# zhouhang95/ray_tracing_in_one_weekend

Measured on AMD Instinct MI355X. Metric: Mray/s (primary+secondary) at 1920x1080/256spp, higher is better.
Workload: dtype f32

## Files before the change

### include/rtow_mi355x_debug.h

```cpp
#ifndef RTOW_MI355X_DEBUG_H
#define RTOW_MI355X_DEBUG_H

#include "rtow_mi355x.h"

#ifdef __cplusplus
extern "C" {
#endif

#define RT_FLAG_TIME_DEPTHS 4u
#define RT_FLAG_PRODUCTION_KERNELS 8u

int rt_get_depth_timings(RtCtx* ctx, uint32_t max_n, float* isect_ms, float* shade_ms, uint64_t* rays);

int rt_debug_render_parts(const RtCtx* ctx, char* buf, uint32_t cap);

enum RtDebugOption {
    RT_OPT_TREE_PLACEMENT = 0,
    RT_OPT_PRIMARY_LISTS = 1,
    RT_OPT_PIXEL_ORDER = 2,
    RT_OPT_TEXEL_POOL = 3,
    RT_OPT_GRID = 4,
    RT_OPT_GRID_CELL = 5,
    RT_OPT_CHAINS = 6,
    RT_OPT_GENERAL_KERNELS = 7,
    RT_OPT_GENERAL_LDS = 8,
    RT_OPT_QUEUE_SHARDS = 9,
    RT_OPT_ISECT_WORKGROUPS = 10,
    RT_OPT_MATERIALISE_PRIMARIES = 11,
    RT_OPT_MEDIUM_SEARCH = 12,
    RT_OPT_POOL_CHUNK_DELAY_US = 13,
    RT_OPT__COUNT = 14
};
int rt_debug_set_option(RtCtx* ctx, uint32_t option, uint32_t value);
int rt_debug_get_option(const RtCtx* ctx, uint32_t option, uint32_t* value);

typedef struct RtSceneInfo {
    uint32_t n_entries;
    uint32_t n_tree_nodes, tree_depth;
    uint32_t tree_in_lds;
    uint32_t general_kernels;
    uint32_t closest_hit_lds_bytes;
    uint32_t grid;
    uint32_t grid_cells[3];
    uint32_t grid_refs;
    uint32_t grid_always;
    uint32_t grid_lds_bytes;
    float grid_cell_size[3];
    uint32_t general_tables_in_lds;
    uint32_t nest;
} RtSceneInfo;
int rt_debug_scene_info(const RtCtx* ctx, RtSceneInfo* info);

int rt_debug_planar_info(const RtCtx* ctx, uint32_t* n_planar, uint32_t* plane_data_in_lds);
int rt_debug_planar_bounds(const RtQuads* quads, float world_mag, float* box, float* slack);

int rt_debug_grid_build(const RtFlatScene* scene, uint32_t cell_per_mille, uint32_t lds_budget, float grid[8], uint32_t dims[3],
                        uint32_t* cells, uint32_t* n_cells, uint16_t* refs, uint32_t* n_refs, uint32_t large[4], uint32_t* n_large);

int rt_debug_world_bounds(const RtFlatScene* scene, float* prim_box, float* prim_box_padded, float* world_sphere, uint32_t* n_entries,
                          uint32_t* entry_id, float* entry_box_padded, float* entry_bs);

int rt_debug_motion_bounds(const RtCtx* ctx, float* entry_box_padded, float* entry_sphere, uint32_t* entry_id, uint32_t entry_cap, uint32_t* n_entries,
                           float grid[6], uint32_t dims[3], uint32_t* cell_begin, uint32_t* cell_id, uint32_t cell_cap, uint32_t* n_cell_ids);

#ifdef RT_PROFILE_LANES
int rt_debug_lane_stats(unsigned long long* out24, int reset);
#endif

typedef struct RtBounceIO {
    uint32_t n;
    uint32_t depth;
    const float* in_o;
    const float* in_d;
    const uint32_t* in_key;
    int32_t* out_hit;
    float* out_t;
    float* out_radiance;
    float* out_attenuation;
    float* out_o;
    float* out_d;
    uint8_t* out_alive;
    uint32_t flags;
} RtBounceIO;
int rt_debug_bounce(RtCtx* ctx, const RtBounceIO* io);

#define RT_ARITH_SHARED_DIVISION 0u
#define RT_ARITH_SQRT 1u
#define RT_ARITH_TO_I32 2u
#define RT_ARITH_TO_U32 3u
int rt_debug_arithmetic(RtCtx* ctx, uint32_t op, uint32_t n, const float* x, const float* a, float* out);


#ifdef __cplusplus
}
#endif
#endif
```

### ray_tracing_in_one_weekend_amd/_ffi.py

```python
import ctypes as C
import os

_PKG_DIR = os.path.dirname(os.path.abspath(__file__))
GPU_LIB_PATH = os.environ.get("RTOW_GPU_LIB") or os.path.join(_PKG_DIR, "librtow_mi355x.so")
HOST_LIB_PATH = os.path.join(_PKG_DIR, "librtow_host.so")

RT_NO_TEX = 0xFFFFFFFF
ERR_INVALID, ERR_DEVICE, ERR_NOMEM, ERR_UNSUPPORTED, ERR_STATE = 1, 2, 3, 4, 5
FLAG_BRUTE_FORCE = 1
FLAG_RUSSIAN_ROULETTE = 2
FLAG_TIME_DEPTHS = 4
FLAG_PRODUCTION_KERNELS = 8
RTH_INVALID = 0xFFFFFFFF

(MAT_EMISSION, MAT_DIFFUSE, MAT_LAMBERT, MAT_METAL, MAT_DIELECTRIC, MAT_ISOTROPIC, MAT_OREN_NAYAR,
 MAT_BURLEY_DIFFUSE, MAT_ROUGH_PLASTIC, MAT_DISNEY_DIFFUSE, MAT_DISNEY_METAL, MAT_DISNEY_SHEEN,
 MAT_DISNEY_CLEARCOAT) = range(13)
TEX_CONSTANT, TEX_CHECKER, TEX_PERLIN, TEX_IMAGE = range(4)
RECT_YZ, RECT_XZ, RECT_XY = range(3)
XF_TRANSLATE, XF_ROTATE_Y = range(2)
NO_XFORM = 0xFFFFFFFF
SKY_GRADIENT, SKY_BLACK, SKY_ENV = range(3)

_f = C.POINTER(C.c_float)
_u8 = C.POINTER(C.c_uint8)
_u16 = C.POINTER(C.c_uint16)
_u32 = C.POINTER(C.c_uint32)
_u64 = C.POINTER(C.c_uint64)


class RtFlatScene(C.Structure):
    _fields_ = [
        ("n_spheres", C.c_uint32),
        ("sph_cx", _f), ("sph_cy", _f), ("sph_cz", _f), ("sph_r", _f), ("sph_mat", _u32),
        ("n_rects", C.c_uint32),
        ("rect_axis", _u8), ("rect_min", _f), ("rect_max", _f), ("rect_mat", _u32),
        ("n_xforms", C.c_uint32),
        ("xf_type", _u8), ("xf_param", _f), ("xf_parent", _u32), ("sph_xform", _u32), ("rect_xform", _u32),
        ("n_media", C.c_uint32),
        ("med_neg_inv_density", _f), ("med_mat", _u32), ("sph_medium", _u32), ("rect_medium", _u32), ("med_xform", _u32),
        ("n_materials", C.c_uint32),
        ("mat_type", _u8), ("mat_color", _f), ("mat_p0", _f), ("mat_p1", _f), ("mat_p2", _f), ("mat_p3", _f),
        ("mat_tex0", _u32), ("mat_tex1", _u32),
        ("n_textures", C.c_uint32),
        ("tex_type", _u8), ("tex_color0", _f), ("tex_color1", _f), ("tex_scale", _f), ("tex_aux", _u32),
        ("n_perlin", C.c_uint32),
        ("perlin_vec", _f), ("perlin_perm", _u16),
        ("n_images", C.c_uint32),
        ("img_w", _u32), ("img_h", _u32), ("img_offset", _u64), ("texels", _f), ("n_texel_floats", C.c_uint64),
        ("sky_type", C.c_uint32), ("sky_image", C.c_uint32),
    ]


class RtCamera(C.Structure):
    _fields_ = [("origin", C.c_float * 3), ("horizontal", C.c_float * 3), ("vertical", C.c_float * 3),
                ("lower_left_corner", C.c_float * 3)]


class RtLens(C.Structure):
    _fields_ = [("lens_radius", C.c_float), ("focus_dist", C.c_float)]


class RtMotion(C.Structure):
    _fields_ = [("n_moving", C.c_uint32), ("sphere", C.POINTER(C.c_uint32)), ("center1", C.POINTER(C.c_float)),
                ("shutter_open", C.c_float), ("shutter_close", C.c_float)]


class RtQuads(C.Structure):
    _fields_ = [("n", C.c_uint32), ("q", C.POINTER(C.c_float)), ("u", C.POINTER(C.c_float)), ("v", C.POINTER(C.c_float)),
                ("kind", C.POINTER(C.c_uint8)), ("mat", C.POINTER(C.c_uint32))]


PLANAR_QUAD, PLANAR_TRIANGLE = 0, 1
PLANAR_MIN_SIN2 = 2.0 ** -20
PLANAR_REACH = 16.0


class RtParams(C.Structure):
    _fields_ = [("nx", C.c_uint32), ("ny", C.c_uint32), ("spp", C.c_uint32), ("max_depth", C.c_int32),
                ("seed", C.c_uint64), ("shard_band", C.c_uint32), ("shard_count", C.c_uint32),
                ("shard_id", C.c_uint32), ("spp_slice", C.c_uint32), ("flags", C.c_uint32), ("reserved", C.c_uint32)]


class RtStats(C.Structure):
    _fields_ = [("n_paths", C.c_uint64), ("n_rays", C.c_uint64), ("n_rays_secondary", C.c_uint64),
                ("n_texture_fetches", C.c_uint64), ("n_bad_dir", C.c_uint64), ("seconds_total", C.c_double),
                ("seconds_trace", C.c_double), ("seconds_device", C.c_double), ("bytes_algorithmic", C.c_uint64),
                ("bytes_trace_algorithmic", C.c_uint64), ("n_trace_launches", C.c_uint32), ("n_slices", C.c_uint32),
                ("rays_per_depth", C.c_uint64 * 64)]

    def as_dict(self):
        d = {k: getattr(self, k) for k, _ in self._fields_ if k != "rays_per_depth"}
        d["rays_per_depth"] = list(self.rays_per_depth)
        return d


class RtBounceIO(C.Structure):
    _fields_ = [("n", C.c_uint32), ("depth", C.c_uint32), ("in_o", _f), ("in_d", _f), ("in_key", _u32),
                ("out_hit", C.POINTER(C.c_int32)), ("out_t", _f), ("out_radiance", _f), ("out_attenuation", _f),
                ("out_o", _f), ("out_d", _f), ("out_alive", _u8), ("flags", C.c_uint32)]


RtProgressFn = C.CFUNCTYPE(None, C.c_void_p, C.c_uint32, C.c_uint32, C.POINTER(C.c_uint8), C.c_uint32, C.c_uint32)

MULTI_COPY_GATHER = 1
(OPT_TREE_PLACEMENT, OPT_PRIMARY_LISTS, OPT_PIXEL_ORDER, OPT_TEXEL_POOL, OPT_GRID, OPT_GRID_CELL, OPT_CHAINS,
 OPT_GENERAL_KERNELS, OPT_GENERAL_LDS, OPT_QUEUE_SHARDS, OPT_ISECT_WORKGROUPS, OPT_MATERIALISE_PRIMARIES, OPT_MEDIUM_SEARCH, OPT_POOL_CHUNK_DELAY_US) = range(14)
OPT_NAMES = {"tree_placement": OPT_TREE_PLACEMENT, "primary_lists": OPT_PRIMARY_LISTS, "pixel_order": OPT_PIXEL_ORDER,
             "texel_pool": OPT_TEXEL_POOL, "grid": OPT_GRID, "grid_cell": OPT_GRID_CELL, "chains": OPT_CHAINS,
             "general_kernels": OPT_GENERAL_KERNELS, "general_lds": OPT_GENERAL_LDS, "queue_shards": OPT_QUEUE_SHARDS,
             "isect_workgroups": OPT_ISECT_WORKGROUPS, "materialise_primaries": OPT_MATERIALISE_PRIMARIES,
             "medium_search": OPT_MEDIUM_SEARCH, "pool_chunk_delay_us": OPT_POOL_CHUNK_DELAY_US}


class RtSceneInfo(C.Structure):
    _fields_ = [("n_entries", C.c_uint32), ("n_tree_nodes", C.c_uint32), ("tree_depth", C.c_uint32), ("tree_in_lds", C.c_uint32),
                ("general_kernels", C.c_uint32), ("closest_hit_lds_bytes", C.c_uint32), ("grid", C.c_uint32),
                ("grid_cells", C.c_uint32 * 3), ("grid_refs", C.c_uint32), ("grid_always", C.c_uint32),
                ("grid_lds_bytes", C.c_uint32), ("grid_cell_size", C.c_float * 3), ("general_tables_in_lds", C.c_uint32), ("nest", C.c_uint32)]

    def as_dict(self):
        d = {k: getattr(self, k) for k, _ in self._fields_ if k not in ("grid_cells", "grid_cell_size")}
        d["grid_cells"], d["grid_cell_size"] = list(self.grid_cells), [float(x) for x in self.grid_cell_size]
        return d


EXPECTED_ABI = 11
GPU_SYMBOLS = ["rt_abi_version", "rt_build_id", "rt_ctx_create", "rt_ctx_destroy", "rt_last_error", "rt_scene_upload",
               "rt_shard_rows", "rt_shard_row_to_image_row", "rt_prepare", "rt_render", "rt_render_device", "rt_debug_bounce", "rt_debug_arithmetic",
               "rt_get_depth_timings", "rt_set_progress", "rt_host_alloc", "rt_host_free", "rt_debug_set_option", "rt_debug_get_option",
               "rt_debug_scene_info", "rt_debug_grid_build", "rt_debug_world_bounds", "rt_debug_render_parts", "rt_multi_create", "rt_multi_create_ex", "rt_multi_destroy", "rt_multi_device_count",
               "rt_multi_last_error", "rt_multi_scene_upload", "rt_multi_render", "rt_deinterleave_bands", "rt_set_lens", "rt_multi_set_lens",
               "rt_set_motion", "rt_multi_set_motion", "rt_debug_motion_bounds",
               "rt_set_quads", "rt_multi_set_quads", "rt_debug_planar_info", "rt_debug_planar_bounds"]
HOST_SYMBOLS = ["rth_last_error", "rth_register_image", "rth_rng_reseed", "rth_scene_build", "rth_scene_new",
                "rth_tex_constant", "rth_tex_checker", "rth_tex_perlin", "rth_tex_image", "rth_material",
                "rth_sphere", "rth_rect", "rth_gbox", "rth_translate", "rth_rotate_y", "rth_constant_medium", "rth_hitable_bbox", "rth_set_sky", "rth_set_camera", "rth_scene_finish", "rth_scene_flat",
                "rth_scene_camera", "rth_scene_sphere_name", "rth_scene_free", "rth_png_write", "rth_output_file_name",
                "rth_set_camera_lens", "rth_scene_lens",
                "rth_moving_sphere", "rth_set_camera_shutter", "rth_scene_motion",
                "rth_quad", "rth_triangle", "rth_scene_quads"]

_gpu_lib = None
_host_lib = None


class GpuLibraryMissing(RuntimeError):
    pass


def load_gpu_library():
    global _gpu_lib
    if _gpu_lib is not None:
        return _gpu_lib
    if not os.path.exists(GPU_LIB_PATH):
        raise GpuLibraryMissing(
            f"{GPU_LIB_PATH} is missing: build it with `python -c 'import __graft_entry__ as g; g.build()'` "
            "(hipcc --offload-arch=gfx950).  There is no CPU fallback for the render path.")
    lib = C.CDLL(GPU_LIB_PATH)
    vp = C.c_void_p
    lib.rt_abi_version.restype = C.c_uint32
    if lib.rt_abi_version() != EXPECTED_ABI:
        raise GpuLibraryMissing(f"{GPU_LIB_PATH} has ABI version {lib.rt_abi_version()}, this package expects {EXPECTED_ABI}: "
                                "rebuild it (python -c 'import __graft_entry__ as g; g.build()')")
    lib.rt_build_id.restype = C.c_char_p
    lib.rt_ctx_create.argtypes = [C.c_int, C.POINTER(vp)]
    lib.rt_ctx_create.restype = C.c_int
    lib.rt_ctx_destroy.argtypes = [vp]
    lib.rt_ctx_destroy.restype = None
    lib.rt_last_error.argtypes = [vp]
    lib.rt_last_error.restype = C.c_char_p
    lib.rt_scene_upload.argtypes = [vp, C.POINTER(RtFlatScene)]
    lib.rt_scene_upload.restype = C.c_int
    lib.rt_shard_rows.argtypes = [C.c_uint32] * 4
    lib.rt_shard_rows.restype = C.c_uint32
    lib.rt_shard_row_to_image_row.argtypes = [C.c_uint32] * 4
    lib.rt_shard_row_to_image_row.restype = C.c_uint32
    lib.rt_prepare.argtypes = [vp, C.POINTER(RtParams)]
    lib.rt_prepare.restype = C.c_int
    lib.rt_render.argtypes = [vp, C.POINTER(RtCamera), C.POINTER(RtParams), _f, _u8, C.POINTER(RtStats)]
    lib.rt_render.restype = C.c_int
    lib.rt_render_device.argtypes = [vp, C.POINTER(RtCamera), C.POINTER(RtParams), vp, vp, C.POINTER(RtStats)]
    lib.rt_render_device.restype = C.c_int
    lib.rt_get_depth_timings.argtypes = [vp, C.c_uint32, _f, _f, _u64]
    lib.rt_get_depth_timings.restype = C.c_int
    lib.rt_debug_bounce.argtypes = [vp, C.POINTER(RtBounceIO)]
    lib.rt_debug_bounce.restype = C.c_int
    lib.rt_debug_arithmetic.argtypes = [vp, C.c_uint32, C.c_uint32, C.POINTER(C.c_float), C.POINTER(C.c_float), C.POINTER(C.c_float)]
    lib.rt_debug_arithmetic.restype = C.c_int
    lib.rt_set_progress.argtypes = [vp, RtProgressFn, vp]
    lib.rt_set_progress.restype = C.c_int
    lib.rt_set_lens.argtypes = [vp, C.POINTER(RtLens)]
    lib.rt_set_lens.restype = C.c_int
    lib.rt_multi_set_lens.argtypes = [vp, C.POINTER(RtLens)]
    lib.rt_multi_set_lens.restype = C.c_int
    lib.rt_set_motion.argtypes = [vp, C.POINTER(RtMotion)]
    lib.rt_set_motion.restype = C.c_int
    lib.rt_multi_set_motion.argtypes = [vp, C.POINTER(RtMotion)]
    lib.rt_multi_set_motion.restype = C.c_int
    lib.rt_debug_motion_bounds.argtypes = [vp, vp, vp, vp, C.c_uint32, C.POINTER(C.c_uint32), C.c_float * 6, C.c_uint32 * 3, vp, vp, C.c_uint32,
                                           C.POINTER(C.c_uint32)]
    lib.rt_debug_motion_bounds.restype = C.c_int
    lib.rt_set_quads.argtypes = [vp, C.POINTER(RtQuads)]
    lib.rt_set_quads.restype = C.c_int
    lib.rt_multi_set_quads.argtypes = [vp, C.POINTER(RtQuads)]
    lib.rt_multi_set_quads.restype = C.c_int
    lib.rt_debug_planar_info.argtypes = [vp, C.POINTER(C.c_uint32), C.POINTER(C.c_uint32)]
    lib.rt_debug_planar_info.restype = C.c_int
    lib.rt_debug_planar_bounds.argtypes = [C.POINTER(RtQuads), C.c_float, vp, vp]
    lib.rt_debug_planar_bounds.restype = C.c_int
    lib.rt_host_alloc.argtypes = [C.c_size_t]
    lib.rt_host_alloc.restype = vp
    lib.rt_host_free.argtypes = [vp]
    lib.rt_host_free.restype = None
    lib.rt_debug_set_option.argtypes = [vp, C.c_uint32, C.c_uint32]
    lib.rt_debug_set_option.restype = C.c_int
    lib.rt_debug_get_option.argtypes = [vp, C.c_uint32, _u32]
    lib.rt_debug_get_option.restype = C.c_int
    lib.rt_debug_scene_info.argtypes = [vp, C.POINTER(RtSceneInfo)]
    lib.rt_debug_scene_info.restype = C.c_int
    lib.rt_debug_render_parts.argtypes = [vp, C.c_char_p, C.c_uint32]
    lib.rt_debug_render_parts.restype = C.c_int
    lib.rt_debug_grid_build.argtypes = [C.POINTER(RtFlatScene), C.c_uint32, C.c_uint32, C.c_float * 8, C.c_uint32 * 3, _u32, _u32, _u16, _u32,
                                        C.c_uint32 * 4, _u32]
    lib.rt_debug_grid_build.restype = C.c_int
    lib.rt_debug_world_bounds.argtypes = [C.POINTER(RtFlatScene), _f, _f, _f, _u32, _u32, _f, _f]
    lib.rt_debug_world_bounds.restype = C.c_int
    lib.rt_multi_create.argtypes = [C.POINTER(C.c_int), C.c_int, C.POINTER(vp)]
    lib.rt_multi_create.restype = C.c_int
    lib.rt_multi_create_ex.argtypes = [C.POINTER(C.c_int), C.c_int, C.c_uint32, C.POINTER(vp)]
    lib.rt_multi_create_ex.restype = C.c_int
    lib.rt_multi_destroy.argtypes = [vp]
    lib.rt_multi_destroy.restype = None
    lib.rt_multi_device_count.argtypes = [vp]
    lib.rt_multi_device_count.restype = C.c_int
    lib.rt_multi_last_error.argtypes = [vp]
    lib.rt_multi_last_error.restype = C.c_char_p
    lib.rt_multi_scene_upload.argtypes = [vp, C.POINTER(RtFlatScene)]
    lib.rt_multi_scene_upload.restype = C.c_int
    lib.rt_multi_render.argtypes = [vp, C.POINTER(RtCamera), C.POINTER(RtParams), _f, _u8, C.POINTER(RtStats)]
    lib.rt_multi_render.restype = C.c_int
    lib.rt_deinterleave_bands.argtypes = [vp, vp, C.c_uint32, C.c_uint32, C.c_uint32, C.c_uint32, vp, vp, vp]
    lib.rt_deinterleave_bands.restype = C.c_int
    _gpu_lib = lib
    return lib


def load_host_library():
    global _host_lib
    if _host_lib is not None:
        return _host_lib
    if not os.path.exists(HOST_LIB_PATH):
        raise RuntimeError(f"{HOST_LIB_PATH} is missing: run __graft_entry__.build()")
    lib = C.CDLL(HOST_LIB_PATH)
    vp = C.c_void_p
    f3 = C.c_float * 3
    lib.rth_last_error.restype = C.c_char_p
    lib.rth_register_image.argtypes = [C.c_char_p, C.c_uint32, C.c_uint32, _f]
    lib.rth_register_image.restype = C.c_int
    lib.rth_rng_reseed.argtypes = [C.c_uint64]
    lib.rth_rng_reseed.restype = None
    lib.rth_scene_build.argtypes = [C.c_char_p, C.c_float, C.POINTER(vp)]
    lib.rth_scene_build.restype = C.c_int
    lib.rth_scene_new.argtypes = [C.POINTER(vp)]
    lib.rth_scene_new.restype = C.c_int
    lib.rth_tex_constant.argtypes = [vp, f3]
    lib.rth_tex_constant.restype = C.c_uint32
    lib.rth_tex_checker.argtypes = [vp, f3, f3]
    lib.rth_tex_checker.restype = C.c_uint32
    lib.rth_tex_perlin.argtypes = [vp, C.c_float]
    lib.rth_tex_perlin.restype = C.c_uint32
    lib.rth_tex_image.argtypes = [vp, C.c_char_p]
    lib.rth_tex_image.restype = C.c_uint32
    lib.rth_material.argtypes = [vp, C.c_uint32, C.c_uint32, C.c_uint32, f3, C.c_float * 4]
    lib.rth_material.restype = C.c_uint32
    lib.rth_sphere.argtypes = [vp, f3, C.c_float, C.c_uint32, C.c_char_p]
    lib.rth_sphere.restype = C.c_uint32
    lib.rth_rect.argtypes = [vp, C.c_uint32, f3, f3, C.c_uint32]
    lib.rth_rect.restype = C.c_uint32
    lib.rth_gbox.argtypes = [vp, f3, f3, C.c_uint32]
    lib.rth_gbox.restype = C.c_uint32
    lib.rth_translate.argtypes = [vp, C.c_uint32, f3]
    lib.rth_translate.restype = C.c_uint32
    lib.rth_rotate_y.argtypes = [vp, C.c_uint32, C.c_float]
    lib.rth_rotate_y.restype = C.c_uint32
    lib.rth_constant_medium.argtypes = [vp, C.c_uint32, C.c_float, C.c_uint32]
    lib.rth_constant_medium.restype = C.c_uint32
    lib.rth_hitable_bbox.argtypes = [vp, C.c_uint32, C.c_float * 6]
    lib.rth_hitable_bbox.restype = C.c_int
    lib.rth_set_sky.argtypes = [vp, C.c_uint32, C.c_char_p]
    lib.rth_set_sky.restype = C.c_int
    lib.rth_set_camera.argtypes = [vp, f3, f3, f3, C.c_float, C.c_float]
    lib.rth_set_camera.restype = C.c_int
    lib.rth_scene_finish.argtypes = [vp, C.c_int]
    lib.rth_scene_finish.restype = C.c_int
    lib.rth_scene_flat.argtypes = [vp]
    lib.rth_scene_flat.restype = C.POINTER(RtFlatScene)
    lib.rth_scene_camera.argtypes = [vp, C.POINTER(RtCamera)]
    lib.rth_scene_camera.restype = C.c_int
    lib.rth_set_camera_lens.argtypes = [vp, f3, f3, f3, C.c_float, C.c_float, C.c_float, C.c_float]
    lib.rth_set_camera_lens.restype = C.c_int
    lib.rth_scene_lens.argtypes = [vp, C.POINTER(RtLens)]
    lib.rth_scene_lens.restype = C.c_int
# ... 23 lines not shown
```

### ray_tracing_in_one_weekend_amd/api.py

```python
import ctypes as C

import numpy as np

from . import _ffi
from ._ffi import RtBounceIO, RtCamera, RtFlatScene, RtLens, RtMotion, RtParams, RtQuads, RtStats


class RtError(RuntimeError):
    pass


def _f3(v):
    return (C.c_float * 3)(*[float(x) for x in v])


def _lens_ptr(lens):
    if lens is None:
        return None
    if not isinstance(lens, RtLens):
        lens = RtLens(*[float(x) for x in lens])
    return C.byref(lens)


def make_motion(spheres, center1, shutter=(0.0, 1.0)):
# ... 266 lines not shown
    fs = ptr.contents
    n_prims = fs.n_spheres + fs.n_rects
    cap = n_prims + fs.n_media
    out = {"prim_box": np.zeros((max(n_prims, 1), 2, 3), np.float32), "prim_box_padded": np.zeros((max(n_prims, 1), 2, 3), np.float32),
           "world_sphere": np.zeros((max(fs.n_spheres, 1), 4), np.float32), "entry_id": np.zeros(max(cap, 1), np.uint32),
           "entry_box_padded": np.zeros((max(cap, 1), 2, 3), np.float32), "entry_bs": np.zeros((max(cap, 1), 4), np.float32)}
    fp = lambda a: a.ctypes.data_as(C.POINTER(C.c_float))
    ne = C.c_uint32(cap)
    rc = lib.rt_debug_world_bounds(ptr, fp(out["prim_box"]), fp(out["prim_box_padded"]), fp(out["world_sphere"]), C.byref(ne),
                                   out["entry_id"].ctypes.data_as(C.POINTER(C.c_uint32)), fp(out["entry_box_padded"]), fp(out["entry_bs"]))
    if rc != 0:
        raise RtError(f"rt_debug_world_bounds failed ({rc})")
    for k in ("prim_box", "prim_box_padded"):
        out[k] = out[k][:n_prims]
    out["world_sphere"] = out["world_sphere"][:fs.n_spheres]
    for k in ("entry_id", "entry_box_padded", "entry_bs"):
        out[k] = out[k][:ne.value]
    return out


def make_params(nx, ny, spp, max_depth=50, seed=95, shard_band=0, shard_count=1, shard_id=0, spp_slice=0, flags=0):
    p = RtParams()
    p.flags = flags
    p.nx, p.ny, p.spp, p.max_depth, p.seed = nx, ny, spp, max_depth, seed
    p.shard_band, p.shard_count, p.shard_id, p.spp_slice = shard_band, shard_count, shard_id, spp_slice
    return p


class Renderer:

    def __init__(self, device=0):
        self._lib = _ffi.load_gpu_library()
        self._ctx = C.c_void_p()
        rc = self._lib.rt_ctx_create(device, C.byref(self._ctx))
        if rc != 0:
            raise RtError(f"rt_ctx_create({device}) failed ({rc}): {self._lib.rt_last_error(None).decode()}")
        self.device = device

    def _raise(self, what, rc):
        raise RtError(f"{what} failed ({rc}): {self._lib.rt_last_error(self._ctx).decode()}")

    @property
    def build_id(self):
        return self._lib.rt_build_id().decode()

    def upload(self, scene):
        ptr = scene.flat_ptr if isinstance(scene, Scene) else C.pointer(scene)
        rc = self._lib.rt_scene_upload(self._ctx, ptr)
        if rc != 0:
            self._raise("rt_scene_upload", rc)

    def prepare(self, params):
        rc = self._lib.rt_prepare(self._ctx, C.byref(params))
        if rc != 0:
            self._raise("rt_prepare", rc)

    def set_option(self, option, value):
        opt = _ffi.OPT_NAMES[option] if isinstance(option, str) else int(option)
        rc = self._lib.rt_debug_set_option(self._ctx, opt, int(value))
        if rc != 0:
            self._raise("rt_debug_set_option", rc)

    def get_option(self, option):
        opt = _ffi.OPT_NAMES[option] if isinstance(option, str) else int(option)
        v = C.c_uint32()
        rc = self._lib.rt_debug_get_option(self._ctx, opt, C.byref(v))
        if rc != 0:
            self._raise("rt_debug_get_option", rc)
        return v.value

    def scene_info(self):
        info = _ffi.RtSceneInfo()
        rc = self._lib.rt_debug_scene_info(self._ctx, C.byref(info))
        if rc != 0:
            self._raise("rt_debug_scene_info", rc)
        d = info.as_dict()
        n, lds = C.c_uint32(0), C.c_uint32(0)
        rc = self._lib.rt_debug_planar_info(self._ctx, C.byref(n), C.byref(lds))
        if rc != 0:
            self._raise("rt_debug_planar_info", rc)
        d["n_planar"], d["plane_data_in_lds"] = n.value, lds.value
        return d

    def shard_rows(self, params):
        return self._lib.rt_shard_rows(params.ny, params.shard_band or 1, params.shard_count, params.shard_id)

    def _pinned(self, shape, dtype):
        n = int(np.prod(shape)) * np.dtype(dtype).itemsize
        key = np.dtype(dtype).char
        if not hasattr(self, "_pin"):
            self._pin, self._pin_retired = {}, []
        ptr, size = self._pin.get(key, (None, 0))
        if size < n:
            if ptr:
                self._pin_retired.append(ptr)
            ptr = self._lib.rt_host_alloc(max(n, 1))
            if not ptr:
                raise RtError("rt_host_alloc failed")
            self._pin[key] = (ptr, n)
        buf = (C.c_char * max(n, 1)).from_address(ptr)
        return np.frombuffer(buf, dtype=dtype, count=int(np.prod(shape))).reshape(shape)

    def render(self, camera, params, want_rgb8=False, pinned=False):
        rows = self.shard_rows(params)
        if pinned:
            img = self._pinned((rows, params.nx, 3), np.float32)
            rgb8 = self._pinned((rows, params.nx, 3), np.uint8) if want_rgb8 else None
        else:
            img = np.zeros((rows, params.nx, 3), dtype=np.float32)
            rgb8 = np.zeros((rows, params.nx, 3), dtype=np.uint8) if want_rgb8 else None
        stats = RtStats()
        rc = self._lib.rt_render(self._ctx, C.byref(camera), C.byref(params),
                                 img.ctypes.data_as(C.POINTER(C.c_float)),
                                 rgb8.ctypes.data_as(C.POINTER(C.c_uint8)) if want_rgb8 else None, C.byref(stats))
        if rc != 0:
            self._raise("rt_render", rc)
        return img, rgb8, stats

    def set_progress(self, fn):
        if fn is None:
            self._progress = None
            rc = self._lib.rt_set_progress(self._ctx, _ffi.RtProgressFn(), None)
        else:
            def tramp(_user, done, total, ptr, nx, rows):
                fn(done, total, np.ctypeslib.as_array(ptr, shape=(rows, nx, 3)).copy())
            self._progress = _ffi.RtProgressFn(tramp)
            rc = self._lib.rt_set_progress(self._ctx, self._progress, None)
        if rc != 0:
            self._raise("rt_set_progress", rc)

    def set_lens(self, lens):
        rc = self._lib.rt_set_lens(self._ctx, _lens_ptr(lens))
        if rc != 0:
            self._raise("rt_set_lens", rc)

    def set_motion(self, motion):
        if motion is not None and not isinstance(motion, RtMotion):
            motion = make_motion(*motion)
        rc = self._lib.rt_set_motion(self._ctx, _motion_ptr(motion))
        if rc != 0:
            self._raise("rt_set_motion", rc)
        self._n_moving = motion.n_moving if motion is not None else 0

    def set_quads(self, quads):
        rc = self._lib.rt_set_quads(self._ctx, _quads_ptr(quads))
        if rc != 0:
            self._raise("rt_set_quads", rc)

    def motion_bounds(self):
        n, nc = C.c_uint32(0), C.c_uint32(0)
        grid, dims = (C.c_float * 6)(), (C.c_uint32 * 3)()
        rc = self._lib.rt_debug_motion_bounds(self._ctx, None, None, None, 0, C.byref(n), grid, dims, None, None, 0, C.byref(nc))
        if rc not in (0, -1):
            self._raise("rt_debug_motion_bounds", rc)
        boxes = np.zeros((n.value, 6), np.float32)
        bs = np.zeros((n.value, 4), np.float32)
        ids = np.zeros(n.value, np.uint32)
        cells = np.zeros(max(nc.value, 1), np.uint32)
        begin = np.zeros(getattr(self, "_n_moving", 0) + 1, np.uint32)
        rc = self._lib.rt_debug_motion_bounds(self._ctx, boxes.ctypes.data, bs.ctypes.data, ids.ctypes.data, n.value, C.byref(n), grid, dims,
                                              begin.ctypes.data, cells.ctypes.data, cells.size, C.byref(nc))
        if rc != 0:
            self._raise("rt_debug_motion_bounds", rc)
        return {"entry_box_padded": boxes, "entry_sphere": bs, "entry_id": ids, "grid_min": np.array(grid[0:3], np.float32),
                "grid_cell": np.array(grid[3:6], np.float32), "grid_dims": tuple(dims), "cell_begin": begin, "cell_id": cells[:nc.value]}

# ... 171 lines not shown
```

### ray_tracing_in_one_weekend_amd/csrc/rt_api.hip

```cpp
#include "../../include/rtow_mi355x_debug.h"
#include "rt_kernels.h"
#include "rt_bvh.h"
#include "rt_grid.h"
#include "rt_pool.h"

#include <hip/hip_runtime.h>

#include <algorithm>
#include <chrono>
#include <cmath>
#include <cstdio>
#include <cstdlib>
#include <cstring>
#include <new>
#include <string>
#include <vector>

using namespace rt;

namespace {

thread_local std::string g_create_error;

struct DevBuf {
    void* p = nullptr;
    size_t bytes = 0;
    bool arena = false;
};

}

struct RtCtx {
    int device = 0;
    hipStream_t stream = nullptr;
    hipStream_t stream2 = nullptr;
    std::vector<hipStream_t> parked_streams;
    hipStream_t paired_with = nullptr;
    bool chains_concurrent = true;
    hipEvent_t ev_fork = nullptr, ev_join = nullptr;
    std::string err;
    bool has_scene = false;
    DevScene ds{};
    size_t arena_top = 0;
    DevBuf scene_region;
    size_t scene_used = 0;
    bool scene_measuring = false;
    size_t scene_measure = 0;
    char* h_stage = nullptr;
    WorkPool pool;
    DevBuf acc, counts, totals, out_f32, out_u8, dbg, genp, lists;
    std::vector<hipEvent_t> events;
    std::vector<hipEvent_t> depth_events;
    int timed_depths = 0;
    std::vector<unsigned long long> timed_rays;
    hipEvent_t ev_begin = nullptr, ev_end = nullptr;
    int n_cu = 256;
    size_t lds_limit = 64 * 1024;
    bool use_bvh = false;
    size_t isect_lds = 0;
    bool bvh_in_lds = false;
    bool general_lds = false;
    bool nest = false;
    bool general_kernels = false;
    bool use_grid = false;
    GridParams grid{};
    size_t grid_lds = 0;
    uint32_t opt[RT_OPT__COUNT] = {};
    uint32_t* h_overflow = nullptr;
    long long last_overflow = -1;
    RtLens lens{0.0f, 1.0f};
    struct Search {
        DevScene ds{};
        bool use_bvh = false, bvh_in_lds = false, general_lds = false, use_grid = false;
        size_t isect_lds = 0, grid_lds = 0;
        GridParams grid{};
        bool general_kernels = false;
    } static_search;
    struct Keep {
        std::vector<float4> geo;
        std::vector<PrimBox> eboxes;
        std::vector<uint32_t> entry_ids;
        std::vector<float4> ent_bs;
        std::vector<uint8_t> bare;
        uint32_t bvh_depth = 0;
        std::vector<MatRec> mats;
        std::vector<TexRec> texs;
        std::vector<float4> srec;
        std::vector<uint8_t> raw_class;
        uint32_t sky_type = 0;
        double world_mag = 0.0;
    } keep;
    bool planar = false;
    GenPlanar gplanar{};
    double planar_reach = 0.0;
    DevBuf quads_region;
    bool motion = false;
    GenMotion gmotion{};
    size_t motion_lds = 0;
    DevBuf motion_region;
    struct MotionDebug {
        std::vector<uint32_t> sphere;
        std::vector<PrimBox> eboxes;
        std::vector<float4> ent_bs;
        HostGrid grid;
    } motion_dbg;
    RtProgressFn progress_fn = nullptr;
    void* progress_user = nullptr;
    bool progress_armed = false;
    DevBuf preview_u8;
    std::vector<uint8_t> preview_host;
    std::vector<std::pair<const char*, double>> parts;
    std::chrono::steady_clock::time_point parts_t{};
    void parts_begin() { parts.clear(), parts_t = std::chrono::steady_clock::now(); }
    void mark(const char* what) {
        const auto t = std::chrono::steady_clock::now();
        parts.emplace_back(what, std::chrono::duration<double, std::milli>(t - parts_t).count());
        parts_t = t;
    }
};

namespace {

int fail(RtCtx* ctx, int code, const std::string& msg) {
    if (ctx) ctx->err = msg;
    return code;
}

#define RT_HIP(ctx, expr)                                                                                  \
    do {                                                                                                   \
        hipError_t e__ = (expr);                                                                           \
        if (e__ != hipSuccess) {                                                                           \
            return fail(ctx, e__ == hipErrorOutOfMemory ? RT_ERR_NOMEM : RT_ERR_DEVICE,                    \
                        std::string(#expr) + ": " + hipGetErrorString(e__));                               \
        }                                                                                                  \
    } while (0)

constexpr size_t RT_STAGE_BYTES = 4u << 20;
constexpr size_t RT_ARENA_MAX = 8ull << 30;

void* arena_alloc(RtCtx* ctx, size_t bytes) {
    const size_t off = (ctx->arena_top + 255u) & ~(size_t)255u;
    const size_t need = off + bytes;
    if (need > RT_ARENA_MAX) return nullptr;
    if (pool_request(ctx->pool, need)) return nullptr;
    if (!pool_wait(ctx->pool, need)) return nullptr;
    ctx->arena_top = need;
    return ctx->pool.base + off;
}

int ensure(RtCtx* ctx, DevBuf& b, size_t bytes, bool plain = false) {
// ... 49 lines not shown
    }
    *dev = reinterpret_cast<const T*>(p);
    return RT_OK;
}

bool mat_needs_tex0(uint32_t t) {
    return t == RT_MAT_EMISSION || t == RT_MAT_DIFFUSE || t == RT_MAT_LAMBERT || t == RT_MAT_ISOTROPIC ||
           t == RT_MAT_OREN_NAYAR || t == RT_MAT_BURLEY_DIFFUSE || t == RT_MAT_ROUGH_PLASTIC ||
           t == RT_MAT_DISNEY_DIFFUSE || t == RT_MAT_DISNEY_METAL || t == RT_MAT_DISNEY_SHEEN;
}

bool class_is_light(uint32_t cls, uint32_t sky_type) {
    if (cls == 0) return sky_type != RT_SKY_ENV;
    const uint32_t ty = (cls - 1u) / 4u, tt = (cls - 1u) % 4u;
    return tt == RT_TEX_CONSTANT && ty <= RT_MAT_ISOTROPIC;
}


__global__ void k_spin(unsigned long long ticks, unsigned long long* sink) {
    const unsigned long long t0 = __builtin_amdgcn_s_memtime();
    unsigned long long t = t0;
    for (uint32_t n = 0; n < (1u << 20) && t - t0 < ticks; ++n) {
        __builtin_amdgcn_s_sleep(16);
        t = __builtin_amdgcn_s_memtime();
    }
    if (sink) *sink = t - t0;
}
int ensure_concurrent_chains(RtCtx* ctx, hipStream_t st) {
    if (ctx->paired_with == st) return RT_OK;
    const unsigned long long ticks = 150000ull;
    hipEvent_t e0 = nullptr, e1 = nullptr;
    RT_HIP(ctx, hipEventCreate(&e0));
    RT_HIP(ctx, hipEventCreate(&e1));
    auto timed = [&](bool both, float& ms) -> int {
        RT_HIP(ctx, hipEventRecord(e0, st));
        if (both) {
            RT_HIP(ctx, hipEventRecord(ctx->ev_fork, st));
            RT_HIP(ctx, hipStreamWaitEvent(ctx->stream2, ctx->ev_fork, 0));
            hipLaunchKernelGGL(k_spin, dim3(1), dim3(64), 0, ctx->stream2, ticks, (unsigned long long*)nullptr);
        }
        hipLaunchKernelGGL(k_spin, dim3(1), dim3(64), 0, st, ticks, (unsigned long long*)nullptr);
        if (both) {
            RT_HIP(ctx, hipEventRecord(ctx->ev_join, ctx->stream2));
            RT_HIP(ctx, hipStreamWaitEvent(st, ctx->ev_join, 0));
        }
        RT_HIP(ctx, hipEventRecord(e1, st));
        RT_HIP(ctx, hipStreamSynchronize(st));
        RT_HIP(ctx, hipEventElapsedTime(&ms, e0, e1));
        return RT_OK;
    };
    int rc;
    float one = 0.f, both = 0.f;
    if (!(rc = timed(false, one)) && !(rc = timed(false, one))) {
        for (int attempt = 0;; ++attempt) {
            if ((rc = timed(true, both))) break;
            ctx->chains_concurrent = both < 1.6f * one;
            if (ctx->chains_concurrent || attempt == 6) break;
            hipStream_t fresh = nullptr;
            if (hipStreamCreateWithFlags(&fresh, hipStreamNonBlocking) != hipSuccess) {
                (void)hipGetLastError();
                break;
            }
            ctx->parked_streams.push_back(ctx->stream2);
            ctx->stream2 = fresh;
        }
    }
    (void)hipEventDestroy(e0);
    (void)hipEventDestroy(e1);
    if (!rc) ctx->paired_with = st;
    return rc;
}

struct StepBuffers {
    Queue qi, qo;
    float2* qhit;
    const uint32_t* cin;
    uint32_t* cout;
    float* rad;
    unsigned long long* totals;
    const GenParams* gpd;
    bool lens = false;
    bool motion = false;
    bool planar = false;
};
bool scene_is_general(const RtCtx* ctx) { return ctx->general_kernels; }
bool grid_enabled(const RtCtx* ctx) { return ctx->use_grid && ctx->opt[RT_OPT_GRID] != 1u && !scene_is_general(ctx); }
bool scene_perlin_lds(const RtCtx* ctx) { return ctx->ds.n_perlin > 0 && ctx->ds.n_perlin <= RT_PERLIN_LDS_MAX_SETS; }

void launch_intersect(RtCtx* ctx, hipStream_t sg, bool use_bvh, bool gen, uint32_t grid, const StepBuffers& b, const IntersectParams& ip) {
    const bool rects = scene_is_general(ctx);
    if (use_bvh && !gen && grid_enabled(ctx)) {
        const size_t mlds = ctx->grid_lds + ctx->motion_lds;
        if (b.motion && ctx->grid.ny == 1u) hipLaunchKernelGGL(k_intersect_grid_motion<true>, dim3(grid), dim3(RT_BVH_BLOCK), mlds, sg, ctx->grid, b.qi.a, b.qi.b, b.qhit, b.cin, ip, b.gpd);
        else if (b.motion) hipLaunchKernelGGL(k_intersect_grid_motion<false>, dim3(grid), dim3(RT_BVH_BLOCK), mlds, sg, ctx->grid, b.qi.a, b.qi.b, b.qhit, b.cin, ip, b.gpd);
        else if (ctx->grid.ny == 1u) hipLaunchKernelGGL(k_intersect_grid<true>, dim3(grid), dim3(RT_BVH_BLOCK), ctx->grid_lds, sg, ctx->grid, b.qi.a, b.qi.b, b.qhit, b.cin, ip);
        else hipLaunchKernelGGL(k_intersect_grid<false>, dim3(grid), dim3(RT_BVH_BLOCK), ctx->grid_lds, sg, ctx->grid, b.qi.a, b.qi.b, b.qhit, b.cin, ip);
        return;
    }
    if (b.planar && use_bvh) {
#define RT_LAUNCH_ISECT_P(G, N, T, L)                                                                                                     \
    hipLaunchKernelGGL((k_intersect<RT_BVH_BLOCK, G, true, N, T, true, L, false, true>), dim3(grid), dim3(RT_BVH_BLOCK), ctx->isect_lds, sg, \
                       ctx->ds, b.qi.a, b.qi.b, b.qhit, b.cin, ip, b.gpd)
#define RT_LAUNCH_ISECT_PT(G, N, L)                          \
    do {                                                     \
        if (ctx->general_lds) RT_LAUNCH_ISECT_P(G, N, true, L); \
        else RT_LAUNCH_ISECT_P(G, N, false, L);              \
    } while (0)
#define RT_LAUNCH_ISECT_PN(G, L)                             \
    do {                                                     \
        if (ctx->bvh_in_lds) RT_LAUNCH_ISECT_PT(G, true, L); \
        else RT_LAUNCH_ISECT_PT(G, false, L);                \
    } while (0)
        if (gen && b.lens) RT_LAUNCH_ISECT_PN(true, true);
        else if (gen) RT_LAUNCH_ISECT_PN(true, false);
        else RT_LAUNCH_ISECT_PN(false, false);
#undef RT_LAUNCH_ISECT_PN
#undef RT_LAUNCH_ISECT_PT
#undef RT_LAUNCH_ISECT_P
        return;
    }
    if (b.planar) {
        hipLaunchKernelGGL(k_intersect_list_planar, dim3(ip.q1 - ip.q0), dim3(256), 0, sg, ctx->ds, b.qi.a, b.qi.b, b.qhit, b.cin, ip, b.gpd);
        return;
    }
#define RT_LAUNCH_ISECT_M(G, R, N, T, X, L)                                                                                      \
    hipLaunchKernelGGL((k_intersect<RT_BVH_BLOCK, G, R, N, T, X, L, true>), dim3(grid), dim3(RT_BVH_BLOCK), ctx->isect_lds, sg, ctx->ds, \
                       b.qi.a, b.qi.b, b.qhit, b.cin, ip, b.gpd)
#define RT_LAUNCH_ISECT_X(G, R, N, T, X)                                                                               \
    do {                                                                                                                \
        if (b.motion && G && b.lens) RT_LAUNCH_ISECT_M(G, R, N, T, X, G);                                               \
        else if (b.motion) RT_LAUNCH_ISECT_M(G, R, N, T, X, false);                                                     \
        else if (G && b.lens)                                                                                                \
            hipLaunchKernelGGL((k_intersect<RT_BVH_BLOCK, G, R, N, T, X, G>), dim3(grid), dim3(RT_BVH_BLOCK), ctx->isect_lds, sg, \
                               ctx->ds, b.qi.a, b.qi.b, b.qhit, b.cin, ip, b.gpd);                                      \
        else                                                                                                            \
            hipLaunchKernelGGL((k_intersect<RT_BVH_BLOCK, G, R, N, T, X>), dim3(grid), dim3(RT_BVH_BLOCK), ctx->isect_lds, sg,  \
                               ctx->ds, b.qi.a, b.qi.b, b.qhit, b.cin, ip, b.gpd);                                      \
    } while (0)
#define RT_LAUNCH_ISECT(G, R, N, T) RT_LAUNCH_ISECT_X(G, R, N, T, false)
#define RT_LAUNCH_ISECT_G(G, N)                       \
    do {                                              \
        if (ctx->nest) {                              \
            if (ctx->general_lds) RT_LAUNCH_ISECT_X(G, true, N, true, true); \
            else RT_LAUNCH_ISECT_X(G, true, N, false, true);      \
        } else if (ctx->general_lds) RT_LAUNCH_ISECT(G, true, N, true); \
        else RT_LAUNCH_ISECT(G, true, N, false);      \
    } while (0)
    if (use_bvh && !ctx->bvh_in_lds && gen) RT_LAUNCH_ISECT_G(true, false);
    else if (use_bvh && !ctx->bvh_in_lds) RT_LAUNCH_ISECT_G(false, false);
    else if (use_bvh && gen && rects) RT_LAUNCH_ISECT_G(true, true);
    else if (use_bvh && gen) RT_LAUNCH_ISECT(true, false, true, false);
    else if (use_bvh && rects) RT_LAUNCH_ISECT_G(false, true);
    else if (use_bvh) RT_LAUNCH_ISECT(false, false, true, false);
#undef RT_LAUNCH_ISECT_G
#undef RT_LAUNCH_ISECT
#undef RT_LAUNCH_ISECT_X
#undef RT_LAUNCH_ISECT_M
    else {
        const size_t list_lds = (size_t)std::min<uint32_t>(std::max<uint32_t>(ctx->ds.n_spheres, 1u), RT_SPHERE_TILE) * sizeof(float4);
        if (b.motion) hipLaunchKernelGGL(k_intersect_list_motion, dim3(ip.q1 - ip.q0), dim3(256), list_lds, sg, ctx->ds, b.qi.a, b.qi.b, b.qhit, b.cin, ip, b.gpd);
        else hipLaunchKernelGGL(k_intersect_list, dim3(ip.q1 - ip.q0), dim3(256), list_lds, sg, ctx->ds, b.qi.a, b.qi.b, b.qhit, b.cin, ip, b.gpd);
    }
}

void launch_shade(RtCtx* ctx, hipStream_t sg, bool gen, bool fused_lists, uint32_t n_shards, const StepBuffers& b, const ShadeParams& sp) {
    const bool rects = scene_is_general(ctx), perlin_lds = scene_perlin_lds(ctx);
    const uint32_t n_fused = (gen && fused_lists) ? ctx->ds.n_spheres * (b.motion ? 2u : 1u) : 0u;
    const size_t shade_lds = shade_lds_bytes(ctx->ds.n_prims + ctx->ds.n_media + (b.planar ? ctx->gplanar.n : 0u), perlin_lds ? ctx->ds.n_perlin : 0u, n_fused, !gen && sp.sort);
    if (b.planar) {
#define RT_LAUNCH_SHADE_P(P, G, L)                                                                                                          \
    hipLaunchKernelGGL((k_shade<P, G, true, true, L, false, true>), dim3(n_shards), dim3(256), shade_lds, sg, ctx->ds, b.qi, b.qhit, b.qo, b.cin, \
                       b.cout, b.rad, sp, b.totals, b.gpd)
#define RT_LAUNCH_SHADE_PP(G, L)                   \
    do {                                           \
        if (perlin_lds) RT_LAUNCH_SHADE_P(true, G, L); \
        else RT_LAUNCH_SHADE_P(false, G, L);       \
    } while (0)
        if (gen && b.lens) RT_LAUNCH_SHADE_PP(true, true);
        else if (gen) RT_LAUNCH_SHADE_PP(true, false);
// ... 331 lines not shown
    ctx->use_grid = false;
    if (ctx->use_bvh && ctx->bvh_in_lds && !general && ctx->opt[RT_OPT_GRID] != 1u) {
        HostGrid hg;
        const size_t half_lds = ctx->lds_limit / 2;
        build_sphere_grid(geo, half_lds > extra ? half_lds - extra : 0u, (double)ctx->opt[RT_OPT_GRID_CELL] * 1e-3, hg, dc);
        if (hg.ok) {
            int rc;
            if ((rc = upload(ctx, hg.cells, &hg.gp.cells)) || (rc = upload(ctx, hg.refs, &hg.gp.refs))) return rc;
            hg.gp.sph_geo = ds.sph_geo;
            ctx->grid = hg.gp;
            ctx->grid_lds = grid_lds_bytes(hg.gp.n_spheres, hg.gp.n_cells, hg.gp.n_refs);
            ctx->use_grid = true;
            if (dc) ctx->motion_dbg.grid = hg;
        }
    }
    ctx->isect_lds += ctx->use_bvh ? ctx->motion_lds : 0u;
    if (!ctx->use_bvh) ctx->motion_lds = 0u;
    return RT_OK;
}

}

extern "C" {

uint32_t rt_abi_version(void) { return RT_ABI_VERSION; }

#ifndef RT_BUILD_ID
#define RT_BUILD_ID "unknown"
#endif
const char* rt_build_id(void) { return RT_BUILD_ID; }

const char* rt_last_error(const RtCtx* ctx) { return ctx ? ctx->err.c_str() : g_create_error.c_str(); }

int rt_ctx_create(int device_id, RtCtx** out_ctx) {
    if (!out_ctx) {
        g_create_error = "rt_ctx_create: out_ctx is NULL";
        return RT_ERR_INVALID;
    }
    *out_ctx = nullptr;
    int n_dev = 0;
    hipError_t e = hipGetDeviceCount(&n_dev);
    if (e != hipSuccess || n_dev <= 0) {
        g_create_error = std::string("rt_ctx_create: no HIP device available (") + hipGetErrorString(e) + ")";
        return RT_ERR_DEVICE;
    }
    if (device_id < 0 || device_id >= n_dev) {
        g_create_error = "rt_ctx_create: device_id out of range";
        return RT_ERR_INVALID;
    }
    RtCtx* ctx = new (std::nothrow) RtCtx();
    if (!ctx) {
        g_create_error = "rt_ctx_create: out of host memory";
        return RT_ERR_NOMEM;
    }
    ctx->device = device_id;
    ctx->pool.device = device_id;
    auto bail = [&](const char* what, hipError_t err) {
        g_create_error = std::string("rt_ctx_create: ") + what + ": " + hipGetErrorString(err);
        if (ctx->h_overflow) (void)hipHostFree(ctx->h_overflow);
        pool_destroy(ctx->pool);
        delete ctx;
        return RT_ERR_DEVICE;
    };
    if ((e = hipSetDevice(device_id)) != hipSuccess) return bail("hipSetDevice", e);
    hipDeviceProp_t prop;
    if ((e = hipGetDeviceProperties(&prop, device_id)) != hipSuccess) return bail("hipGetDeviceProperties", e);
    ctx->n_cu = prop.multiProcessorCount > 0 ? prop.multiProcessorCount : 256;
    ctx->lds_limit = prop.sharedMemPerBlock ? prop.sharedMemPerBlock : 64 * 1024;
    if ((e = hipStreamCreateWithFlags(&ctx->stream, hipStreamNonBlocking)) != hipSuccess) return bail("hipStreamCreate", e);
    {
        const void* variants[] = {
#define RT_ISECT_VARIANTS(G, R, N, T) reinterpret_cast<const void*>(&k_intersect<RT_BVH_BLOCK, G, R, N, T>)
            RT_ISECT_VARIANTS(false, false, true, false), RT_ISECT_VARIANTS(false, true, true, false),
            RT_ISECT_VARIANTS(true, false, true, false),  RT_ISECT_VARIANTS(true, true, true, false),
            RT_ISECT_VARIANTS(false, true, false, false), RT_ISECT_VARIANTS(true, true, false, false),
            RT_ISECT_VARIANTS(false, true, true, true),   RT_ISECT_VARIANTS(true, true, true, true),
            RT_ISECT_VARIANTS(false, true, false, true),  RT_ISECT_VARIANTS(true, true, false, true),
#undef RT_ISECT_VARIANTS
#define RT_ISECT_VARIANTS(G, N, T) reinterpret_cast<const void*>(&k_intersect<RT_BVH_BLOCK, G, true, N, T, true>)
            RT_ISECT_VARIANTS(false, true, false), RT_ISECT_VARIANTS(true, true, false), RT_ISECT_VARIANTS(false, false, false), RT_ISECT_VARIANTS(true, false, false),
            RT_ISECT_VARIANTS(false, true, true),  RT_ISECT_VARIANTS(true, true, true),  RT_ISECT_VARIANTS(false, false, true),  RT_ISECT_VARIANTS(true, false, true),
#undef RT_ISECT_VARIANTS
            reinterpret_cast<const void*>(&k_intersect_grid<true>), reinterpret_cast<const void*>(&k_intersect_grid<false>),
            reinterpret_cast<const void*>(&k_debug_bounce<RT_BVH_BLOCK, true, true>),
            reinterpret_cast<const void*>(&k_debug_bounce<RT_BVH_BLOCK, true, false>),
#define RT_SHADE_VARIANTS(P, G) reinterpret_cast<const void*>(&k_shade<P, G, false>), reinterpret_cast<const void*>(&k_shade<P, G, true>), reinterpret_cast<const void*>(&k_shade<P, G, true, true>)
            RT_SHADE_VARIANTS(true, true), RT_SHADE_VARIANTS(true, false), RT_SHADE_VARIANTS(false, true), RT_SHADE_VARIANTS(false, false),
#undef RT_SHADE_VARIANTS
#define RT_ISECT_LENS(R, N, T, X) reinterpret_cast<const void*>(&k_intersect<RT_BVH_BLOCK, true, R, N, T, X, true>)
            RT_ISECT_LENS(false, true, false, false), RT_ISECT_LENS(true, true, false, false), RT_ISECT_LENS(true, true, true, false),
            RT_ISECT_LENS(true, false, false, false), RT_ISECT_LENS(true, false, true, false), RT_ISECT_LENS(true, true, false, true),
            RT_ISECT_LENS(true, true, true, true),    RT_ISECT_LENS(true, false, false, true), RT_ISECT_LENS(true, false, true, true),
#undef RT_ISECT_LENS
#define RT_SHADE_LENS(P) reinterpret_cast<const void*>(&k_shade<P, true, false, false, true>), reinterpret_cast<const void*>(&k_shade<P, true, true, false, true>), \
                         reinterpret_cast<const void*>(&k_shade<P, true, true, true, true>)
            RT_SHADE_LENS(true), RT_SHADE_LENS(false),
#undef RT_SHADE_LENS
#define RT_ISECT_MOTION(R, N, T, X)                                                                     \
    reinterpret_cast<const void*>(&k_intersect<RT_BVH_BLOCK, false, R, N, T, X, false, true>),          \
        reinterpret_cast<const void*>(&k_intersect<RT_BVH_BLOCK, true, R, N, T, X, false, true>),       \
        reinterpret_cast<const void*>(&k_intersect<RT_BVH_BLOCK, true, R, N, T, X, true, true>)
            RT_ISECT_MOTION(false, true, false, false), RT_ISECT_MOTION(true, true, false, false), RT_ISECT_MOTION(true, true, true, false),
            RT_ISECT_MOTION(true, false, false, false), RT_ISECT_MOTION(true, false, true, false), RT_ISECT_MOTION(true, true, false, true),
            RT_ISECT_MOTION(true, true, true, true),    RT_ISECT_MOTION(true, false, false, true), RT_ISECT_MOTION(true, false, true, true),
#undef RT_ISECT_MOTION
#define RT_SHADE_MOTION(P, R, X)                                                                                                           \
    reinterpret_cast<const void*>(&k_shade<P, false, R, X, false, true>), reinterpret_cast<const void*>(&k_shade<P, true, R, X, false, true>), \
        reinterpret_cast<const void*>(&k_shade<P, true, R, X, true, true>)
            RT_SHADE_MOTION(true, false, false), RT_SHADE_MOTION(true, true, false), RT_SHADE_MOTION(true, true, true),
            RT_SHADE_MOTION(false, false, false), RT_SHADE_MOTION(false, true, false), RT_SHADE_MOTION(false, true, true),
#undef RT_SHADE_MOTION
            reinterpret_cast<const void*>(&k_intersect_grid_motion<true>), reinterpret_cast<const void*>(&k_intersect_grid_motion<false>),
            reinterpret_cast<const void*>(&k_debug_bounce_motion<RT_BVH_BLOCK, true, true>),
            reinterpret_cast<const void*>(&k_debug_bounce_motion<RT_BVH_BLOCK, true, false>),
#define RT_ISECT_PLANAR(N, T)                                                                                   \
    reinterpret_cast<const void*>(&k_intersect<RT_BVH_BLOCK, false, true, N, T, true, false, false, true>),     \
        reinterpret_cast<const void*>(&k_intersect<RT_BVH_BLOCK, true, true, N, T, true, false, false, true>),  \
        reinterpret_cast<const void*>(&k_intersect<RT_BVH_BLOCK, true, true, N, T, true, true, false, true>)
            RT_ISECT_PLANAR(true, true), RT_ISECT_PLANAR(true, false), RT_ISECT_PLANAR(false, true), RT_ISECT_PLANAR(false, false),
#undef RT_ISECT_PLANAR
#define RT_SHADE_PLANAR(P)                                                                   \
    reinterpret_cast<const void*>(&k_shade<P, false, true, true, false, false, true>),       \
        reinterpret_cast<const void*>(&k_shade<P, true, true, true, false, false, true>),    \
        reinterpret_cast<const void*>(&k_shade<P, true, true, true, true, false, true>)
            RT_SHADE_PLANAR(true), RT_SHADE_PLANAR(false),
#undef RT_SHADE_PLANAR
            reinterpret_cast<const void*>(&k_debug_bounce_planar<RT_BVH_BLOCK, true, true>),
            reinterpret_cast<const void*>(&k_debug_bounce_planar<RT_BVH_BLOCK, true, false>),
        };
        for (const void* fn : variants)
            if ((e = hipFuncSetAttribute(fn, hipFuncAttributeMaxDynamicSharedMemorySize, (int)ctx->lds_limit)) != hipSuccess)
                return bail("hipFuncSetAttribute(MaxDynamicSharedMemorySize)", e);
    }
    if ((e = hipStreamCreateWithFlags(&ctx->stream2, hipStreamNonBlocking)) != hipSuccess) return bail("hipStreamCreate", e);
    if ((e = hipEventCreateWithFlags(&ctx->ev_fork, hipEventDisableTiming)) != hipSuccess) return bail("hipEventCreate", e);
    if ((e = hipEventCreateWithFlags(&ctx->ev_join, hipEventDisableTiming)) != hipSuccess) return bail("hipEventCreate", e);
    if ((e = hipEventCreate(&ctx->ev_begin)) != hipSuccess) return bail("hipEventCreate", e);
    if ((e = hipEventCreate(&ctx->ev_end)) != hipSuccess) return bail("hipEventCreate", e);
    if ((e = hipHostMalloc((void**)&ctx->h_overflow, sizeof(uint32_t), hipHostMallocDefault)) != hipSuccess) return bail("hipHostMalloc", e);
    if ((e = hipHostMalloc((void**)&ctx->h_stage, RT_STAGE_BYTES, hipHostMallocDefault)) != hipSuccess) return bail("hipHostMalloc", e);
    (void)pool_request(ctx->pool, 256u << 20);
    *out_ctx = ctx;
    return RT_OK;
}

void rt_ctx_destroy(RtCtx* ctx) {
    if (!ctx) return;
    (void)hipSetDevice(ctx->device);
    if (ctx->stream) (void)hipStreamSynchronize(ctx->stream);
    if (ctx->stream2) (void)hipStreamSynchronize(ctx->stream2);
    free_scene(ctx);
    free_buf(ctx->scene_region);
    free_buf(ctx->acc), free_buf(ctx->counts), free_buf(ctx->totals);
    free_buf(ctx->out_f32), free_buf(ctx->out_u8), free_buf(ctx->dbg), free_buf(ctx->genp);
    free_buf(ctx->preview_u8), free_buf(ctx->lists);
    free_buf(ctx->motion_region), free_buf(ctx->quads_region);
    for (auto ev : ctx->events) (void)hipEventDestroy(ev);
    for (auto ev : ctx->depth_events) (void)hipEventDestroy(ev);
    if (ctx->ev_begin) (void)hipEventDestroy(ctx->ev_begin);
    if (ctx->ev_end) (void)hipEventDestroy(ctx->ev_end);
    if (ctx->ev_fork) (void)hipEventDestroy(ctx->ev_fork);
    if (ctx->ev_join) (void)hipEventDestroy(ctx->ev_join);
    if (ctx->stream2) (void)hipStreamDestroy(ctx->stream2);
    for (auto sp : ctx->parked_streams) (void)hipStreamDestroy(sp);
    if (ctx->stream) (void)hipStreamDestroy(ctx->stream);
    if (ctx->h_overflow) (void)hipHostFree(ctx->h_overflow);
// ... 377 lines not shown
    }
    ctx->static_search = RtCtx::Search{ctx->ds, ctx->use_bvh, ctx->bvh_in_lds, ctx->general_lds, ctx->use_grid, ctx->isect_lds, ctx->grid_lds, ctx->grid,
                                       ctx->general_kernels};
    return RT_OK;
}

static GenLens host_gen_lens(const RtCamera* cam, const RtLens& lens) {
    GenLens g{};
    const double R = lens.lens_radius;
    double H[3], V[3], O[3], L[3];
    for (int k = 0; k < 3; ++k) H[k] = cam->horizontal[k], V[k] = cam->vertical[k], O[k] = cam->origin[k], L[k] = cam->lower_left_corner[k];
    const double hn = std::sqrt((H[0] * H[0] + H[1] * H[1]) + H[2] * H[2]), vn = std::sqrt((V[0] * V[0] + V[1] * V[1]) + V[2] * V[2]);
    for (int k = 0; k < 3; ++k) g.lu[k] = (float)(R * H[k] / hn), g.lv[k] = (float)(R * V[k] / vn);
    g.focus_dist = lens.focus_dist;
    double lu2 = 0.0, lv2 = 0.0, luv = 0.0, mu = 0.0, mv = 0.0, mo = 0.0;
    for (int k = 0; k < 3; ++k) {
        const double a = g.lu[k], b = g.lv[k];
        lu2 += a * a, lv2 += b * b, luv += a * b;
        mu = std::max(mu, std::fabs(a)), mv = std::max(mv, std::fabs(b)), mo = std::max(mo, std::fabs(O[k]));
    }
    const double ulp = 1.0 / 16777216.0;
    const double off = std::sqrt((1.0 + 1.0 / 4194304.0) * (std::max(lu2, lv2) + std::fabs(luv)));
    const double grow = (off + 1.7321 * (3.0 * ulp * (mu + mv) + ulp * (mo + off))) * (1.0 + 1e-6);
    const double n[3] = {H[1] * V[2] - H[2] * V[1], H[2] * V[0] - H[0] * V[2], H[0] * V[1] - H[1] * V[0]};
    const double h = std::fabs((L[0] - O[0]) * n[0] + (L[1] - O[1]) * n[1] + (L[2] - O[2]) * n[2]) / std::sqrt(n[0] * n[0] + n[1] * n[1] + n[2] * n[2]);
    double st = grow / ((double)lens.focus_dist * h) * (1.0 + 1e-6);
    if (!(st <= 0.5)) st = 1.0;
    g.grow = std::nextafter((float)grow, INFINITY);
    g.sin_tilt = std::nextafter((float)st, INFINITY);
    return g;
}

static int check_params(RtCtx* ctx, const RtCamera* cam, const RtParams* p) {
    if (!ctx) return RT_ERR_INVALID;
    if (!ctx->has_scene) return fail(ctx, RT_ERR_STATE, "render: no scene uploaded");
    if (!cam || !p) return fail(ctx, RT_ERR_INVALID, "render: camera/params NULL");
    if (p->nx == 0 || p->ny == 0 || p->spp == 0) return fail(ctx, RT_ERR_INVALID, "render: nx, ny and spp must be > 0");
    if (p->max_depth < 0 || p->max_depth > 4096) return fail(ctx, RT_ERR_INVALID, "render: max_depth out of range [0, 4096]");
    if ((uint64_t)p->nx * p->ny > 0xFFFFFFFFull) return fail(ctx, RT_ERR_INVALID, "render: image too large");
    if (p->shard_count > 1 && p->shard_id >= p->shard_count) return fail(ctx, RT_ERR_INVALID, "render: shard_id >= shard_count");
    if (rt_shard_rows(p->ny, p->shard_band ? p->shard_band : 1u, p->shard_count, p->shard_id) >= (1u << 21))
        return fail(ctx, RT_ERR_UNSUPPORTED, "render: a shard of 2^21 or more image rows is not supported");
    return RT_OK;
}

static int render_impl(RtCtx* ctx, const RtCamera* cam, const RtParams* prm, void* d_out_rgb_f32, void* d_out_rgb8,
                       void* stream_v, RtStats* stats, float* h_out_f32 = nullptr, uint8_t* h_out_u8 = nullptr) {
    int rc = check_params(ctx, cam, prm);
    if (rc) return rc;
    if (ctx->planar) {
        const double lens_r = ctx->lens.lens_radius > 0.0f ? (double)ctx->lens.lens_radius : 0.0;
        for (int k = 0; k < 3; ++k)
            if (!(std::fabs((double)cam->origin[k]) + lens_r <= ctx->planar_reach))
                return fail(ctx, RT_ERR_UNSUPPORTED, "render: the camera lies outside RT_PLANAR_REACH x W = " + std::to_string(ctx->planar_reach) +
                                                         " of the scene with its planar primitives (rtow_mi355x.h): the culling bound of rt_set_quads does not cover it");
    }
    RT_HIP(ctx, hipSetDevice(ctx->device));
    hipStream_t st = stream_v ? (hipStream_t)stream_v : ctx->stream;
    const auto wall0 = std::chrono::steady_clock::now();
    ctx->parts_begin();
    ctx->last_overflow = -1;

    const uint32_t nx = prm->nx, ny = prm->ny, spp = prm->spp;
    const uint32_t band = prm->shard_band ? prm->shard_band : 1u;
    const uint32_t scount = prm->shard_count <= 1 ? 1u : prm->shard_count;
    const uint32_t rows = rt_shard_rows(ny, band, scount, prm->shard_id);
    const uint64_t npix64 = (uint64_t)rows * nx;
    if (npix64 == 0) {
        if (stats) std::memset(stats, 0, sizeof(*stats));
        return RT_OK;
    }
    const uint32_t npix = (uint32_t)npix64;
    const int n_depths = prm->max_depth + 1;
    const uint32_t nq = queue_shards(ctx);
    const bool use_bvh = ctx->use_bvh && !(prm->flags & RT_FLAG_BRUTE_FORCE);
    const bool fuse_gen = use_bvh && ctx->opt[RT_OPT_MATERIALISE_PRIMARIES] != 1u;
    const bool want_lists = use_bvh && fuse_gen && spp >= 4 && ctx->ds.n_entries > 0 && ctx->ds.n_entries <= 2048 && ctx->opt[RT_OPT_PRIMARY_LISTS] != 1u &&
                            !ctx->planar;

    ctx->pool.chunk_delay_us.store(ctx->opt[RT_OPT_POOL_CHUNK_DELAY_US]);
    if ((rc = ensure(ctx, ctx->acc, (size_t)npix * 3 * sizeof(float)))) return rc;
    const size_t counts_bytes = (size_t)(n_depths + 1) * nq * sizeof(uint32_t);
    if ((rc = ensure(ctx, ctx->counts, counts_bytes))) return rc;
    const size_t totals_bytes = (size_t)(n_depths + 2) * sizeof(unsigned long long);
    if ((rc = ensure(ctx, ctx->totals, totals_bytes))) return rc;
    if ((rc = ensure(ctx, ctx->genp, sizeof(GenParams) + RT_PLANAR_OFFSET + sizeof(GenPlanar)))) return rc;
    if (want_lists &&(rc = ensure(ctx, ctx->lists, ((size_t)npix + 1u) * sizeof(uint4)))) return rc;
    GenParams* gpd = (GenParams*)ctx->genp.p;
    float* acc = (float*)ctx->acc.p;
    uint32_t* counts = (uint32_t*)ctx->counts.p;
    unsigned long long* totals = (unsigned long long*)ctx->totals.p;
    SlicePlan plan;
    if ((rc = plan_slices(ctx, prm, npix64, plan))) return rc;
    if (const char* e = pool_request(ctx->pool, plan.want_bytes)) return fail(ctx, RT_ERR_NOMEM, std::string("render: ") + e);
    const size_t wbase = work_base(ctx);
    const uint32_t isect_grid = queue_geom(ctx, npix * plan.S_cap).isect_grid;
    ctx->mark("small_buffers_and_pool_request");

    if (nq >= 2u * RT_ISECT_MAX_SHARDS && (rc = ensure_concurrent_chains(ctx, st))) return rc;
    ctx->mark("queue_probe");
    RT_HIP(ctx, hipEventRecord(ctx->ev_begin, st));
    RT_HIP(ctx, hipMemsetAsync(acc, 0, (size_t)npix * 3 * sizeof(float), st));
    RT_HIP(ctx, hipMemsetAsync(totals, 0, totals_bytes, st));

    GenParams gp{};
    for (int k = 0; k < 3; ++k) {
        gp.cam_origin[k] = cam->origin[k];
        gp.cam_horizontal[k] = cam->horizontal[k];
        gp.cam_vertical[k] = cam->vertical[k];
        gp.cam_llc[k] = cam->lower_left_corner[k];
    }
    gp.nx = nx, gp.ny = ny, gp.npix = npix;
    gp.shard_band = band, gp.shard_count = scount, gp.shard_id = prm->shard_id;
    gp.nq = nq, gp.cap = 0u;
    gp.seed_lo = (uint32_t)prm->seed, gp.seed_hi = (uint32_t)(prm->seed >> 32);
    gp.lists = nullptr;
    gp.n_overflow = nullptr;
    const bool lens = ctx->lens.lens_radius > 0.0f;
    const GenLens glens = lens ? host_gen_lens(cam, ctx->lens) : GenLens{};
    bool no_overflow = false;
    {
        auto inv = [](uint32_t d) { return (float)((1.0 / (double)d) * (1.0 - 1.0 / 4194304.0)); };
        gp.inv_npix = inv(npix), gp.inv_nx = inv(nx), gp.inv_band = inv(band);
        const uint32_t po = ctx->opt[RT_OPT_PIXEL_ORDER];
        const bool want_tiles = po ? po == 2u : !scene_is_general(ctx);
        gp.tiles_per_row = (nx % 8u == 0u && rows >= 8u && want_tiles) ? nx / 8u : 0u;
        gp.tile_pixels = gp.tiles_per_row * 64u * (rows / 8u);
        gp.inv_tpr = gp.tiles_per_row ? inv(gp.tiles_per_row) : 0.0f;
    }
    if (want_lists) {
        gp.lists = (const uint4*)ctx->lists.p;
        uint32_t* n_overflow = (uint32_t*)((uint4*)ctx->lists.p + npix);
        gp.n_overflow = n_overflow;
        RT_HIP(ctx, hipMemsetAsync(n_overflow, 0, sizeof(uint4), st));
        const size_t lists_lds = (size_t)ctx->ds.n_entries * sizeof(float4) + 4u * RT_LIST_WAVE_CAP * 2u;
        if (lens)
            hipLaunchKernelGGL(k_primary_lists<true>, dim3((npix + 255u) / 256u), dim3(256), lists_lds, st, ctx->ds, gp, (uint4*)ctx->lists.p, n_overflow, glens);
        else
            hipLaunchKernelGGL(k_primary_lists<false>, dim3((npix + 255u) / 256u), dim3(256), lists_lds, st, ctx->ds, gp, (uint4*)ctx->lists.p, n_overflow, glens);
        if (!scene_is_general(ctx)) {
            RT_HIP(ctx, hipMemcpyAsync(ctx->h_overflow, n_overflow, sizeof(uint32_t), hipMemcpyDeviceToHost, st));
            RT_HIP(ctx, hipStreamSynchronize(st));
            no_overflow = *ctx->h_overflow == 0u;
            ctx->last_overflow = *ctx->h_overflow;
        }
        ctx->mark("primary_lists_and_in_frame_sync");
    }

    uint32_t n_trace_launches = 0;
    const bool time_depths = (prm->flags & RT_FLAG_TIME_DEPTHS) != 0;
    ctx->timed_depths = 0;
    if (time_depths) {
        while (ctx->depth_events.size() < 3 * (size_t)n_depths) {
            hipEvent_t ev;
            RT_HIP(ctx, hipEventCreate(&ev));
            ctx->depth_events.push_back(ev);
        }
    }
    IntersectParams ip{nq, 0u, 0, 0u, nq};
    const uint32_t chains_opt = ctx->opt[RT_OPT_CHAINS];
    const bool one_chain = chains_opt ? chains_opt == 1u : (ctx->ds.n_xforms > 0 || ctx->ds.n_media > 0 || (use_bvh && !ctx->bvh_in_lds));
    const uint32_t n_groups = (nq >= 2u * RT_ISECT_MAX_SHARDS && !time_depths && !one_chain) ? 2u : 1u;
    const uint32_t shards_per_wg = (nq + isect_grid - 1u) / isect_grid;
    const bool rects = scene_is_general(ctx);
    uint32_t n_slices = 0, s0 = 0;
    const uint32_t S_progress = std::min(plan.S_cap, std::max(1u, (spp + 31u) / 32u));
    double pool_wait_ms = 0.0;
    while (s0 < spp) {
        const uint32_t sl = n_slices;
        const uint32_t sc_max = std::min(plan.S_cap, spp - s0);
        uint32_t sc = 0;
        for (;;) {
            const size_t mapped = ctx->pool.mapped.load();
            const uint32_t fits = slice_fit(ctx, npix, mapped > wbase ? mapped - wbase : 0u, sc_max);
            if (fits >= sc_max) { sc = sc_max; break; }
            const bool growing = pool_growing(ctx->pool);
            if (!growing) {
                if (ctx->pool.mapped.load() != mapped) continue;
                if (fits == 0u) return fail(ctx, RT_ERR_NOMEM, "render: no device memory for the work buffers of one sample per pixel (" +
                                                                    std::to_string(slice_bytes(ctx, npix, 1u) >> 20) + " MB): " + pool_error(ctx->pool));
                sc = fits;
                break;
            }
            const bool device_idle = sl == 0u || hipEventQuery(ctx->events[2 * (size_t)sl - 1]) == hipSuccess;
            if (plan.by_library && fits >= std::min(S_progress, sc_max) && device_idle) { sc = fits; break; }
            const auto tw = std::chrono::steady_clock::now();
            pool_wait_progress(ctx->pool, mapped, 200u);
            pool_wait_ms += std::chrono::duration<double, std::milli>(std::chrono::steady_clock::now() - tw).count();
        }
        (void)hipGetLastError();
        const uint32_t n_max = npix * sc;
        const uint32_t cap = queue_geom(ctx, n_max).cap;
        const WorkView wv = work_view(ctx, work_layout((size_t)nq * cap, n_max), wbase);
        const Queue* Q = wv.Q;
        float2* qhit = wv.qhit;
        float* rad = wv.rad;
        gp.cap = cap, ip.cap = cap;
        while (ctx->events.size() < 2 * (size_t)(sl + 1u)) {
            hipEvent_t ev;
            RT_HIP(ctx, hipEventCreate(&ev));
            ctx->events.push_back(ev);
        }
        ++n_slices;
        gp.s0 = s0;
        gp.n_rays = npix * sc;
        RT_HIP(ctx, hipMemsetAsync(counts, 0, counts_bytes, st));
        if (ctx->motion) hipLaunchKernelGGL(k_set_motion, dim3(1), dim3(64), 0, st, gpd, ctx->gmotion);
        if (ctx->planar) hipLaunchKernelGGL(k_set_planar, dim3(1), dim3(64), 0, st, gpd, ctx->gplanar);
        if (lens) hipLaunchKernelGGL(k_init_counts<true>, dim3((nq + 255u) / 256u), dim3(256), 0, st, gp, counts, gpd, glens);
        else hipLaunchKernelGGL(k_init_counts<false>, dim3((nq + 255u) / 256u), dim3(256), 0, st, gp, counts, gpd, glens);
        if (!fuse_gen && lens) hipLaunchKernelGGL(k_gen_primary<true>, dim3((gp.n_rays + 255u) / 256u), dim3(256), 0, st, gp, Q[0], glens);
        else if (!fuse_gen) hipLaunchKernelGGL(k_gen_primary<false>, dim3((gp.n_rays + 255u) / 256u), dim3(256), 0, st, gp, Q[0], glens);
        RT_HIP(ctx, hipEventRecord(ctx->events[2 * sl], st));
        if (n_groups > 1u) {
            RT_HIP(ctx, hipEventRecord(ctx->ev_fork, st));
            RT_HIP(ctx, hipStreamWaitEvent(ctx->stream2, ctx->ev_fork, 0));
        }
        for (int depth = 0; depth < n_depths; ++depth)
        for (uint32_t grp = 0; grp < n_groups; ++grp) {
            hipStream_t sg = grp ? ctx->stream2 : st;
            const uint32_t q0 = grp * (nq / n_groups), q1 = grp + 1u == n_groups ? nq : q0 + nq / n_groups;
            const uint32_t isect_grid_g = (q1 - q0 + shards_per_wg - 1u) / shards_per_wg;
            const Queue& qi = Q[depth & 1];
            const Queue& qo = Q[(depth + 1) & 1];
            const uint32_t* cin = counts + (size_t)depth * nq;
            uint32_t* cout = counts + (size_t)(depth + 1) * nq;
            const bool td = time_depths && sl == 0;
            if (td) RT_HIP(ctx, hipEventRecord(ctx->depth_events[3 * (size_t)depth], st));
            const bool gen = fuse_gen && depth == 0;
            ip.depth = depth;
            ip.q0 = q0, ip.q1 = q1;
            const StepBuffers sb{qi, qo, qhit, cin, cout, rad, totals, gpd, lens, ctx->motion, ctx->planar};
            const bool no_primary_trace = gen && !rects && gp.lists != nullptr && no_overflow;
            if (!no_primary_trace) launch_intersect(ctx, sg, use_bvh, gen, isect_grid_g, sb, ip);
            if (td) RT_HIP(ctx, hipEventRecord(ctx->depth_events[3 * (size_t)depth + 1], st));
            const ShadeParams sp{nq, cap, depth, prm->max_depth, depth > 0 ? 1u : 0u,
                                 (prm->flags & RT_FLAG_RUSSIAN_ROULETTE) ? 1u : 0u, q0};
            launch_shade(ctx, sg, gen, !rects && gp.lists != nullptr, q1 - q0, sb, sp);
            if (td) RT_HIP(ctx, hipEventRecord(ctx->depth_events[3 * (size_t)depth + 2], st));
            if (grp == 0u) n_trace_launches += no_primary_trace ? 1u : 2u;
        }
        if (n_groups > 1u) {
            RT_HIP(ctx, hipEventRecord(ctx->ev_join, ctx->stream2));
            RT_HIP(ctx, hipStreamWaitEvent(st, ctx->ev_join, 0));
        }
        if (time_depths && sl == 0) {
            ctx->timed_depths = n_depths;
            ctx->timed_rays.assign((size_t)n_depths, 0ull);
            std::vector<uint32_t> hc((size_t)(n_depths + 1) * nq);
            RT_HIP(ctx, hipMemcpyAsync(hc.data(), counts, hc.size() * sizeof(uint32_t), hipMemcpyDeviceToHost, st));
            RT_HIP(ctx, hipStreamSynchronize(st));
            for (int d = 0; d < n_depths; ++d)
                for (uint32_t k = 0; k < nq; ++k) ctx->timed_rays[(size_t)d] += hc[(size_t)d * nq + k];
        }
        RT_HIP(ctx, hipEventRecord(ctx->events[2 * sl + 1], st));
        hipLaunchKernelGGL(k_resolve, dim3((npix + 255u) / 256u), dim3(256), 0, st, rad, acc, npix, sc);
        hipLaunchKernelGGL(k_accum_counts, dim3((unsigned)n_depths), dim3(256), 0, st, counts, nq, (uint32_t)n_depths, totals + 2);
        if (ctx->progress_armed && ctx->progress_fn && s0 + sc < spp) {
            const uint32_t done = s0 + sc;
            hipLaunchKernelGGL(k_finalize, dim3((npix + 255u) / 256u), dim3(256), 0, st, acc, (float*)nullptr,
                               (uint8_t*)ctx->preview_u8.p, nx, rows, done, gp.tiles_per_row, gp.tile_pixels);
            RT_HIP(ctx, hipMemcpyAsync(ctx->preview_host.data(), ctx->preview_u8.p, (size_t)npix * 3, hipMemcpyDeviceToHost, st));
            RT_HIP(ctx, hipStreamSynchronize(st));
            ctx->progress_fn(ctx->progress_user, done, spp, ctx->preview_host.data(), nx, rows);
        }
        s0 += sc;
    }
    if (pool_wait_ms > 0.0) ctx->parts.emplace_back("of_which_waiting_for_the_pool", pool_wait_ms);
    hipLaunchKernelGGL(k_finalize, dim3((npix + 255u) / 256u), dim3(256), 0, st, acc, (float*)d_out_rgb_f32,
                       (uint8_t*)d_out_rgb8, nx, rows, spp, gp.tiles_per_row, gp.tile_pixels);
    RT_HIP(ctx, hipEventRecord(ctx->ev_end, st));
    RT_HIP(ctx, hipGetLastError());
    ctx->mark("enqueue_all_launches");
    if (h_out_f32) RT_HIP(ctx, hipMemcpyAsync(h_out_f32, d_out_rgb_f32, (size_t)npix * 3 * sizeof(float), hipMemcpyDeviceToHost, st));
    if (h_out_u8) RT_HIP(ctx, hipMemcpyAsync(h_out_u8, d_out_rgb8, (size_t)npix * 3, hipMemcpyDeviceToHost, st));
    if ((h_out_f32 || h_out_u8) && !stats) RT_HIP(ctx, hipStreamSynchronize(st));

    if (stats) {
        RT_HIP(ctx, hipStreamSynchronize(st));
        ctx->mark("wait_for_the_device");
        std::vector<unsigned long long> h((size_t)n_depths + 2);
        RT_HIP(ctx, hipMemcpy(h.data(), totals, totals_bytes, hipMemcpyDeviceToHost));
        std::memset(stats, 0, sizeof(*stats));
        stats->n_paths = (uint64_t)npix * spp;
        stats->n_texture_fetches = h[0];
        stats->n_bad_dir = h[1];
        for (int d = 0; d < n_depths; ++d) {
            stats->n_rays += h[(size_t)d + 2];
            if (d < 64) stats->rays_per_depth[d] = h[(size_t)d + 2];
        }
        stats->n_rays_secondary = stats->n_rays - std::min(stats->n_rays, stats->n_paths);
        float ms = 0.0f;
        double trace_ms = 0.0;
        for (uint32_t sl = 0; sl < n_slices; ++sl) {
            RT_HIP(ctx, hipEventElapsedTime(&ms, ctx->events[2 * sl], ctx->events[2 * sl + 1]));
            trace_ms += ms;
        }
        RT_HIP(ctx, hipEventElapsedTime(&ms, ctx->ev_begin, ctx->ev_end));
        stats->seconds_trace = trace_ms * 1e-3;
        stats->seconds_device = ms * 1e-3;
        stats->bytes_algorithmic = 96ull * stats->n_rays + 24ull * stats->n_paths + 12ull * stats->n_texture_fetches;
        stats->bytes_trace_algorithmic = 48ull * stats->n_rays + 48ull * stats->n_rays_secondary + 12ull * stats->n_paths +
                                         12ull * stats->n_texture_fetches;
        stats->n_trace_launches = n_trace_launches;
        stats->n_slices = n_slices;
        stats->seconds_total = std::chrono::duration<double>(std::chrono::steady_clock::now() - wall0).count();
    }
    return RT_OK;
}

int rt_prepare(RtCtx* ctx, const RtParams* prm) {
    if (!ctx) return RT_ERR_INVALID;
    if (!prm || prm->nx == 0 || prm->ny == 0 || prm->spp == 0) return fail(ctx, RT_ERR_INVALID, "rt_prepare: params NULL, or nx, ny or spp 0");
    if (prm->shard_count > 1 && prm->shard_id >= prm->shard_count) return fail(ctx, RT_ERR_INVALID, "rt_prepare: shard_id >= shard_count");
    RT_HIP(ctx, hipSetDevice(ctx->device));
    const uint64_t npix64 = (uint64_t)rt_shard_rows(prm->ny, prm->shard_band ? prm->shard_band : 1u, prm->shard_count, prm->shard_id) * prm->nx;
    if (npix64 == 0) return RT_OK;
    if (npix64 > 0xFFFFFFFFull) return fail(ctx, RT_ERR_INVALID, "rt_prepare: image too large");
    SlicePlan plan;
    int rc = plan_slices(ctx, prm, npix64, plan);
    if (rc) return rc;
    ctx->pool.chunk_delay_us.store(ctx->opt[RT_OPT_POOL_CHUNK_DELAY_US]);
    const size_t small = (size_t)npix64 * 48u + (64u << 20);
    if (const char* e = pool_request(ctx->pool, plan.want_bytes + small)) return fail(ctx, RT_ERR_NOMEM, std::string("rt_prepare: ") + e);
    return RT_OK;
}

int rt_render_device(RtCtx* ctx, const RtCamera* cam, const RtParams* prm, void* d_out_rgb_f32, void* stream_v,
                     RtStats* stats) {
    if (ctx && !d_out_rgb_f32) return fail(ctx, RT_ERR_INVALID, "rt_render_device: output pointer is NULL");
    return render_impl(ctx, cam, prm, d_out_rgb_f32, nullptr, stream_v, stats);
}

int rt_render(RtCtx* ctx, const RtCamera* cam, const RtParams* prm, float* out_rgb_f32, uint8_t* out_rgb8, RtStats* stats) {
    int rc = check_params(ctx, cam, prm);
    if (rc) return rc;
    RT_HIP(ctx, hipSetDevice(ctx->device));
    const uint32_t band = prm->shard_band ? prm->shard_band : 1u;
    const uint32_t rows = rt_shard_rows(prm->ny, band, prm->shard_count, prm->shard_id);
    const size_t n = (size_t)rows * prm->nx * 3;
    if ((rc = ensure(ctx, ctx->out_f32, n * sizeof(float)))) return rc;
    if (out_rgb8 && (rc = ensure(ctx, ctx->out_u8, n))) return rc;
    if (ctx->progress_fn) {
        if ((rc = ensure(ctx, ctx->preview_u8, n))) return rc;
        ctx->preview_host.resize(n);
    }
    RtStats local;
    ctx->progress_armed = true;
    rc = render_impl(ctx, cam, prm, ctx->out_f32.p, out_rgb8 ? ctx->out_u8.p : nullptr, nullptr, stats ? stats : &local,
                     n ? out_rgb_f32 : nullptr, n ? out_rgb8 : nullptr);
    ctx->progress_armed = false;
    return rc;
}

void* rt_host_alloc(size_t bytes) {
    void* p = nullptr;
    if (hipHostMalloc(&p, bytes ? bytes : 1, hipHostMallocDefault) != hipSuccess) {
        (void)hipGetLastError();
        return nullptr;
    }
    return p;
}

void rt_host_free(void* p) {
// ... 471 lines not shown
    const uint32_t n_tex = (uint32_t)kp.texs.size();
    for (uint32_t i = 0; i < n; ++i) {
        const MatRec& m = kp.mats[quads->mat[i]];
        const bool has_t0 = mat_needs_tex0(m.type) && m.tex0 < n_tex;
        const uint32_t tt = has_t0 ? kp.texs[m.tex0].type : 0u;
        sclass[base + i] = (uint8_t)(1u + m.type * 4u + tt);
        const size_t r = 5 * (size_t)(base + i);
        srec[r + 1] = make_float4(fbits(m.type), fbits(tt), fbits(has_t0 ? kp.texs[m.tex0].aux : 0u), fbits(m.tex1));
        srec[r + 2] = has_t0 ? make_float4(kp.texs[m.tex0].c0r, kp.texs[m.tex0].c0g, kp.texs[m.tex0].c0b, m.p0) : make_float4(m.cr, m.cg, m.cb, m.p0);
        srec[r + 3] = make_float4(m.p1, m.p2, has_t0 ? kp.texs[m.tex0].scale : 0.0f, fbits(m.tex0));
    }
    bool class_present[RT_NCLASS] = {};
    class_present[0] = true;
    for (uint8_t c : sclass) class_present[c] = true;
    uint32_t class_key[RT_NCLASS] = {}, n_keys = 0;
    for (int pass = 0; pass < 2; ++pass)
        for (uint32_t c = 0; c < RT_NCLASS; ++c)
            if (class_present[c] && class_is_light(c, kp.sky_type) == (pass == 0)) class_key[c] = n_keys++;
    for (uint8_t& c : sclass) c = (uint8_t)class_key[c];
    std::vector<PrimBox> eboxes = kp.eboxes;
    std::vector<uint32_t> entry_ids = kp.entry_ids;
    for (uint32_t i = 0; i < n; ++i) eboxes.push_back(ph.boxes[i]), entry_ids.push_back(base + i);
    HostBvh bvh;
    build_prim_bvh(eboxes, RT_BVH_MAX_DEPTH, bvh);
    for (auto& dd : bvh.d) {
        if (dd.x < 0 && dd.x != INT_MIN) dd.x = ~(int)entry_ids[(size_t)~dd.x];
        if (dd.y < 0 && dd.y != INT_MIN) dd.y = ~(int)entry_ids[(size_t)~dd.y];
    }
    HostBvh4 bvh4;
    collapse_bvh4(bvh, bvh4);
    if (bvh4.id.size() >= 32768u || bvh.depth > RT_BVH_MAX_DEPTH) return fail(ctx, RT_ERR_INVALID, "rt_set_quads: the tree over the set has more nodes or levels than the kernels index");
    RT_HIP(ctx, hipDeviceSynchronize());
    DevScene ds = ctx->static_search.ds;
    ds.n_bvh4_nodes = (uint32_t)bvh4.id.size();
    ds.bvh4_depth = bvh4.depth;
    ds.n_entries = (uint32_t)eboxes.size();
    ds.key_miss = class_key[0];
    {
        double ext2 = 0.0;
        for (int k = 0; k < 3; ++k) {
            float lo = FLT_MAX, hi = -FLT_MAX;
            for (const PrimBox& b : eboxes) lo = std::min(lo, b.mn[k]), hi = std::max(hi, b.mx[k]);
            if (hi > lo) ext2 += ((double)hi - lo) * ((double)hi - lo);
        }
        ds.bvh_exact_eps = (float)(std::sqrt(ext2) / 1024.0);
    }
    const float4* d_pq = nullptr;
    auto upload_all = [&]() -> int {
        int rc;
        if ((rc = upload(ctx, ph.pq, &d_pq)) || (rc = upload(ctx, srec, &ds.sph_rec)) || (rc = upload(ctx, sclass, &ds.sph_class)) ||
            (rc = upload(ctx, bvh4.id, &ds.bvh4_id)) || (rc = upload(ctx, bvh4.p[0], &ds.bvh4_p[0])) || (rc = upload(ctx, bvh4.p[1], &ds.bvh4_p[1])) ||
            (rc = upload(ctx, bvh4.p[2], &ds.bvh4_p[2])) || (rc = upload(ctx, bvh4.p[3], &ds.bvh4_p[3])) ||
            (rc = upload(ctx, bvh4.p[4], &ds.bvh4_p[4])) || (rc = upload(ctx, bvh4.p[5], &ds.bvh4_p[5]))) return rc;
        return RT_OK;
    };
    const bool had_set = ctx->planar;
    const DevBuf scene_region = ctx->scene_region;
    const size_t scene_used = ctx->scene_used;
    ctx->scene_measuring = true, ctx->scene_measure = 0;
    (void)upload_all();
    ctx->scene_measuring = false;
    int rc = ensure(ctx, ctx->quads_region, ctx->scene_measure + (1u << 20));
    if (!rc) {
        ctx->scene_region = ctx->quads_region, ctx->scene_used = 0;
        rc = upload_all();
        ctx->scene_region = scene_region, ctx->scene_used = scene_used;
    }
    if (rc) {
        const std::string err = ctx->err;
        if (had_set) restore_static_search(ctx);
        ctx->err = err;
        return rc;
    }
    restore_static_search(ctx);
    ctx->ds = ds;
    ctx->gplanar = GenPlanar{d_pq, base, n};
    ctx->planar = true;
    ctx->planar_reach = RT_PLANAR_REACH * ph.world_mag;
    if ((rc = configure_search(ctx, bvh.depth, kp.geo, nullptr))) {
        const std::string err = ctx->err;
        restore_static_search(ctx);
        ctx->err = err;
        return rc;
    }
    return RT_OK;
}

int rt_get_depth_timings(RtCtx* ctx, uint32_t max_n, float* isect_ms, float* shade_ms, uint64_t* rays) {
    if (!ctx) return RT_ERR_INVALID;
    RT_HIP(ctx, hipSetDevice(ctx->device));
    const int n = std::min<int>(ctx->timed_depths, (int)max_n);
    for (int d = 0; d < n; ++d) {
        float a_ms = 0.f, b_ms = 0.f;
        RT_HIP(ctx, hipEventElapsedTime(&a_ms, ctx->depth_events[3 * (size_t)d], ctx->depth_events[3 * (size_t)d + 1]));
        RT_HIP(ctx, hipEventElapsedTime(&b_ms, ctx->depth_events[3 * (size_t)d + 1], ctx->depth_events[3 * (size_t)d + 2]));
        if (isect_ms) isect_ms[d] = a_ms;
        if (shade_ms) shade_ms[d] = b_ms;
        if (rays) rays[d] = ctx->timed_rays[(size_t)d];
    }
    return n;
}

static int debug_bounce_production(RtCtx* ctx, const RtBounceIO* io) {
    const uint32_t n = io->n;
    hipStream_t st = ctx->stream;
    const QueueGeom qg = queue_geom(ctx, n);
    const uint32_t nq = qg.nq, cap = qg.cap;
    int rc;
    if ((rc = ensure(ctx, ctx->counts, (size_t)2 * nq * sizeof(uint32_t)))) return rc;
    if ((rc = ensure(ctx, ctx->totals, 4 * sizeof(unsigned long long)))) return rc;
    if ((rc = ensure(ctx, ctx->genp, sizeof(GenParams) + RT_PLANAR_OFFSET + sizeof(GenPlanar)))) return rc;
    if ((rc = ensure(ctx, ctx->dbg, (size_t)n * 6 * sizeof(float)))) return rc;
    const WorkLayout wl = work_layout((size_t)nq * cap, n);
    const size_t wbase = work_base(ctx);
    if (const char* e = pool_request(ctx->pool, wbase + wl.total)) return fail(ctx, RT_ERR_NOMEM, std::string("rt_debug_bounce: ") + e);
    if (!pool_wait(ctx->pool, wbase + wl.total)) return fail(ctx, RT_ERR_NOMEM, "rt_debug_bounce: no device memory for the work buffers: " + pool_error(ctx->pool));
    const WorkView wv = work_view(ctx, wl, wbase);
    const Queue* Q = wv.Q;
    uint32_t* counts = (uint32_t*)ctx->counts.p;
    float* d_o = (float*)ctx->dbg.p;
    float* d_d = d_o + 3 * (size_t)n;
    RT_HIP(ctx, hipMemcpyAsync(d_o, io->in_o, 3 * (size_t)n * 4, hipMemcpyHostToDevice, st));
    RT_HIP(ctx, hipMemcpyAsync(d_d, io->in_d, 3 * (size_t)n * 4, hipMemcpyHostToDevice, st));
    RT_HIP(ctx, hipMemsetAsync(counts, 0, (size_t)2 * nq * sizeof(uint32_t), st));
    RT_HIP(ctx, hipMemsetAsync(ctx->totals.p, 0, 4 * sizeof(unsigned long long), st));
    RT_HIP(ctx, hipMemsetAsync(wv.rad, 0xFF, (size_t)n * RT_RAD_FLOATS * sizeof(float), st));
    GenParams gp{};
    gp.nx = n, gp.ny = 1, gp.npix = n, gp.n_rays = n, gp.s0 = 0;
    gp.shard_band = 1, gp.shard_count = 1, gp.shard_id = 0;
    gp.nq = nq, gp.cap = cap;
    gp.inv_npix = gp.inv_nx = (float)((1.0 / (double)n) * (1.0 - 1.0 / 4194304.0));
    gp.inv_band = (float)(1.0 - 1.0 / 4194304.0);
    hipLaunchKernelGGL(k_init_counts<false>, dim3((nq + 255u) / 256u), dim3(256), 0, st, gp, counts, (GenParams*)ctx->genp.p, GenLens{});
    if (ctx->motion) hipLaunchKernelGGL(k_set_motion, dim3(1), dim3(64), 0, st, (GenParams*)ctx->genp.p, ctx->gmotion);
    if (ctx->planar) hipLaunchKernelGGL(k_set_planar, dim3(1), dim3(64), 0, st, (GenParams*)ctx->genp.p, ctx->gplanar);
    hipLaunchKernelGGL(k_debug_fill, dim3((n + 255u) / 256u), dim3(256), 0, st, gp, Q[0], d_o, d_d);
    const bool use_bvh = ctx->use_bvh && !(io->flags & RT_FLAG_BRUTE_FORCE);
    const StepBuffers sb{Q[0], Q[1], wv.qhit, counts, counts + nq, wv.rad,
                         (unsigned long long*)ctx->totals.p, (const GenParams*)ctx->genp.p, false, ctx->motion, ctx->planar};
    const IntersectParams ip{nq, cap, (int)io->depth, 0u, nq};
    launch_intersect(ctx, st, use_bvh, false, qg.isect_grid, sb, ip);
    const ShadeParams sp{nq, cap, (int)io->depth, 0x7FFFFFFF, 1u, 0u, 0u};
    launch_shade(ctx, st, false, false, nq, sb, sp);
    RT_HIP(ctx, hipGetLastError());
    std::vector<float4> ha((size_t)nq * cap), hb((size_t)nq * cap);
    std::vector<float> hrad((size_t)n * RT_RAD_FLOATS);
    std::vector<float2> hc((size_t)nq * cap), hh((size_t)nq * cap);
    std::vector<uint32_t> hcnt((size_t)2 * nq);
    RT_HIP(ctx, hipMemcpyAsync(hh.data(), wv.qhit, hh.size() * sizeof(float2), hipMemcpyDeviceToHost, st));
    std::vector<float4> hab;
    if (RT_QSTRIDE == 1u) {
        RT_HIP(ctx, hipMemcpyAsync(ha.data(), Q[1].a, ha.size() * sizeof(float4), hipMemcpyDeviceToHost, st));
        RT_HIP(ctx, hipMemcpyAsync(hb.data(), Q[1].b, hb.size() * sizeof(float4), hipMemcpyDeviceToHost, st));
    } else {
        hab.resize(2 * ha.size());
        RT_HIP(ctx, hipMemcpyAsync(hab.data(), Q[1].a, hab.size() * sizeof(float4), hipMemcpyDeviceToHost, st));
    }
    RT_HIP(ctx, hipMemcpyAsync(hc.data(), Q[1].c, hc.size() * sizeof(float2), hipMemcpyDeviceToHost, st));
    RT_HIP(ctx, hipMemcpyAsync(hrad.data(), wv.rad, hrad.size() * sizeof(float), hipMemcpyDeviceToHost, st));
    RT_HIP(ctx, hipMemcpyAsync(hcnt.data(), counts, hcnt.size() * sizeof(uint32_t), hipMemcpyDeviceToHost, st));
    RT_HIP(ctx, hipStreamSynchronize(st));
    for (size_t i = 0; i < hab.size() / 2; ++i) ha[i] = hab[2 * i], hb[i] = hab[2 * i + 1];
    auto bits = [](float f) {
        uint32_t u;
        std::memcpy(&u, &f, 4);
        return u;
    };
    for (uint32_t i = 0; i < n; ++i) {
        const uint32_t chunk = i >> 8;
        const size_t pos = (size_t)(chunk % nq) * cap + (size_t)(chunk / nq) * 256u + (i & 255u);
        const int hit = (int)bits(hh[pos].y);
        io->out_hit[i] = hit;
        io->out_t[i] = hit >= 0 ? hh[pos].x : 0.0f;
        io->out_alive[i] = 0;
        for (int k = 0; k < 3; ++k) io->out_attenuation[3 * (size_t)i + k] = io->out_o[3 * (size_t)i + k] = io->out_d[3 * (size_t)i + k] = 0.0f;
        for (int c = 0; c < 3; ++c) io->out_radiance[3 * (size_t)i + c] = hrad[RT_RAD_FLOATS * (size_t)i + c];
    }
    size_t n_out = 0;
    for (uint32_t q = 0; q < nq; ++q) {
        if (hcnt[nq + q] > cap) return fail(ctx, RT_ERR_DEVICE, "rt_debug_bounce: shard overflow");
        for (uint32_t k = 0; k < hcnt[nq + q]; ++k, ++n_out) {
            const size_t pos = (size_t)q * cap + k;
            const uint32_t slot = bits(ha[pos].w);
            if (slot >= n || io->out_alive[slot]) return fail(ctx, RT_ERR_DEVICE, "rt_debug_bounce: bad or repeated slot in the output queue");
            io->out_alive[slot] = 1;
            io->out_o[3 * (size_t)slot] = ha[pos].x, io->out_o[3 * (size_t)slot + 1] = ha[pos].y, io->out_o[3 * (size_t)slot + 2] = ha[pos].z;
            io->out_d[3 * (size_t)slot] = hb[pos].x, io->out_d[3 * (size_t)slot + 1] = hb[pos].y, io->out_d[3 * (size_t)slot + 2] = hb[pos].z;
            io->out_attenuation[3 * (size_t)slot] = hb[pos].w, io->out_attenuation[3 * (size_t)slot + 1] = hc[pos].x, io->out_attenuation[3 * (size_t)slot + 2] = hc[pos].y;
            for (int c = 0; c < 3; ++c) io->out_radiance[3 * (size_t)slot + c] = 0.0f;
        }
    }
    return RT_OK;
}

int rt_debug_bounce(RtCtx* ctx, const RtBounceIO* io) {
    if (!ctx) return RT_ERR_INVALID;
    if (!ctx->has_scene) return fail(ctx, RT_ERR_STATE, "rt_debug_bounce: no scene uploaded");
    if (!io || !io->in_o || !io->in_d || !io->in_key || !io->out_hit || !io->out_t || !io->out_radiance ||
        !io->out_attenuation || !io->out_o || !io->out_d || !io->out_alive)
        return fail(ctx, RT_ERR_INVALID, "rt_debug_bounce: NULL array");
    if (io->n == 0) return RT_OK;
    RT_HIP(ctx, hipSetDevice(ctx->device));
    if (io->flags & RT_FLAG_PRODUCTION_KERNELS) return debug_bounce_production(ctx, io);
    const size_t n = io->n;
    const size_t off_o = 0, off_d = off_o + 3 * n, off_key = off_d + 3 * n, off_hit = off_key + 2 * n, off_t = off_hit + n,
                 off_rad = off_t + n, off_att = off_rad + 3 * n, off_so = off_att + 3 * n, off_sd = off_so + 3 * n,
                 off_alive = off_sd + 3 * n, total = off_alive + (n + 3) / 4 + 4;
    int rc;
    if ((rc = ensure(ctx, ctx->dbg, total * 4))) return rc;
    float* base = (float*)ctx->dbg.p;
    hipStream_t st = ctx->stream;
    RT_HIP(ctx, hipMemcpyAsync(base + off_o, io->in_o, 3 * n * 4, hipMemcpyHostToDevice, st));
    RT_HIP(ctx, hipMemcpyAsync(base + off_d, io->in_d, 3 * n * 4, hipMemcpyHostToDevice, st));
    RT_HIP(ctx, hipMemcpyAsync(base + off_key, io->in_key, 2 * n * 4, hipMemcpyHostToDevice, st));
    const bool use_bvh = ctx->use_bvh && !(io->flags & RT_FLAG_BRUTE_FORCE);
#define RT_DEBUG_BOUNCE(B, U, L, LDS)                                                                                                      \
    do {                                                                                                                                   \
        if (ctx->planar)                                                                                                                   \
            hipLaunchKernelGGL((k_debug_bounce_planar<B, U, L>), dim3((unsigned)((n + B - 1) / B)), dim3(B), LDS, st, ctx->ds, (uint32_t)n, \
                               (int)io->depth, base + off_o, base + off_d, (const uint32_t*)(base + off_key), (int*)(base + off_hit),      \
                               base + off_t, base + off_rad, base + off_att, base + off_so, base + off_sd, (uint8_t*)(base + off_alive),   \
                               ctx->gplanar);                                                                                              \
        else if (ctx->motion)                                                                                                              \
            hipLaunchKernelGGL((k_debug_bounce_motion<B, U, L>), dim3((unsigned)((n + B - 1) / B)), dim3(B), LDS, st, ctx->ds, (uint32_t)n, \
                               (int)io->depth, base + off_o, base + off_d, (const uint32_t*)(base + off_key), (int*)(base + off_hit),      \
                               base + off_t, base + off_rad, base + off_att, base + off_so, base + off_sd, (uint8_t*)(base + off_alive),   \
                               ctx->gmotion);                                                                                              \
        else                                                                                                                               \
            hipLaunchKernelGGL((k_debug_bounce<B, U, L>), dim3((unsigned)((n + B - 1) / B)), dim3(B), LDS, st, ctx->ds, (uint32_t)n,       \
                               (int)io->depth, base + off_o, base + off_d, (const uint32_t*)(base + off_key), (int*)(base + off_hit),      \
                               base + off_t, base + off_rad, base + off_att, base + off_so, base + off_sd, (uint8_t*)(base + off_alive));  \
    } while (0)
    if (use_bvh && !ctx->bvh_in_lds) {
        RT_DEBUG_BOUNCE(RT_BVH_BLOCK, true, false, ctx->isect_lds);
    } else if (use_bvh) {
        RT_DEBUG_BOUNCE(RT_BVH_BLOCK, true, true, ctx->isect_lds);
    } else {
        const size_t lds_bytes = (size_t)std::min<uint32_t>(std::max<uint32_t>(ctx->ds.n_spheres, 1u), RT_SPHERE_TILE) * sizeof(float4);
        RT_DEBUG_BOUNCE(256, false, true, lds_bytes);
    }
#undef RT_DEBUG_BOUNCE
    RT_HIP(ctx, hipGetLastError());
    RT_HIP(ctx, hipMemcpyAsync(io->out_hit, base + off_hit, n * 4, hipMemcpyDeviceToHost, st));
    RT_HIP(ctx, hipMemcpyAsync(io->out_t, base + off_t, n * 4, hipMemcpyDeviceToHost, st));
    RT_HIP(ctx, hipMemcpyAsync(io->out_radiance, base + off_rad, 3 * n * 4, hipMemcpyDeviceToHost, st));
    RT_HIP(ctx, hipMemcpyAsync(io->out_attenuation, base + off_att, 3 * n * 4, hipMemcpyDeviceToHost, st));
    RT_HIP(ctx, hipMemcpyAsync(io->out_o, base + off_so, 3 * n * 4, hipMemcpyDeviceToHost, st));
    RT_HIP(ctx, hipMemcpyAsync(io->out_d, base + off_sd, 3 * n * 4, hipMemcpyDeviceToHost, st));
    RT_HIP(ctx, hipMemcpyAsync(io->out_alive, base + off_alive, n, hipMemcpyDeviceToHost, st));
    RT_HIP(ctx, hipStreamSynchronize(st));
    return RT_OK;
}

}
// ... 46 lines not shown
```

### ray_tracing_in_one_weekend_amd/csrc/rt_grid.h

```cpp
#pragma once
#include "rt_kernels.h"

#include <algorithm>
#include <cmath>
#include <vector>

namespace rt {

#define RT_GRID_MAX_ALWAYS 4u
#define RT_GRID_CNT_BITS 12u
#define RT_GRID_CNT_MASK 0xFFFu
#define RT_GRID_MAX_SPHERES 4095u
#ifndef RT_GRID_BIG_CELLS
#define RT_GRID_BIG_CELLS 64.0
#endif
#ifndef RT_GRID_MAX_CELLS
#define RT_GRID_MAX_CELLS 16384u
#endif
#ifndef RT_GRID_CELL_FACTOR
#define RT_GRID_CELL_FACTOR 1.4
#endif
#ifndef RT_GRID_REFILL_MIN
#define RT_GRID_REFILL_MIN RT_REFILL_MIN
#endif
// ... 84 lines not shown
            if (!(pad >= 4.0 * steps * (std::sqrt(diag2) + maxabs) / 8388608.0) || !(pad * 1048576.0 >= 2.0 * maxabs)) continue;
        }
        g.nx = dims[0], g.ny = dims[1], g.nz = dims[2];
        g.n_cells = (uint32_t)total;
        auto cell_range = [&](uint32_t i, int k, uint32_t& a, uint32_t& b) {
            const double c = k == 0 ? sph[i].x : (k == 1 ? sph[i].y : sph[i].z), r = 0.5 * diam[i] + pad;
            const double fa = std::floor((c + std::min(disp(i, k), 0.0) - r - (double)g.g0[k]) / (double)g.cs[k]),
                         fb = std::floor((c + std::max(disp(i, k), 0.0) + r - (double)g.g0[k]) / (double)g.cs[k]);
            a = (uint32_t)std::min<double>(std::max(fa, 0.0), dims[k] - 1.0);
            b = (uint32_t)std::min<double>(std::max(fb, 0.0), dims[k] - 1.0);
        };
        auto reaches = [&](uint32_t i, uint32_t x, uint32_t y, uint32_t z) {
            if (moves(i)) return true;
            const double c[3] = {sph[i].x, sph[i].y, sph[i].z}, r = 0.5 * diam[i] + pad;
            const uint32_t q[3] = {x, y, z};
            double d2 = 0.0;
            for (int k = 0; k < 3; ++k) {
                const double mn = (double)g.g0[k] + (double)g.cs[k] * q[k], mx = mn + (double)g.cs[k];
                const double e = c[k] < mn ? mn - c[k] : (c[k] > mx ? c[k] - mx : 0.0);
                d2 += e * e;
            }
            return d2 <= r * r;
        };
        std::vector<uint32_t> count(g.n_cells, 0u);
        out.cells.clear();
        for (int pass = 0; pass < 2; ++pass) {
            if (pass == 1) {
                uint64_t sum = 0;
                bool bad = false;
                out.cells.assign(g.n_cells, 0u);
                for (uint32_t c = 0; c < g.n_cells; ++c) {
                    if (count[c] > RT_GRID_CNT_MASK) bad = true;
                    out.cells[c] = (uint32_t)(sum << RT_GRID_CNT_BITS);
                    sum += count[c];
                }
                if (bad || sum + n + 1u >= (1u << (32u - RT_GRID_CNT_BITS))) {
                    out.cells.clear();
                    break;
                }
                out.refs.assign((size_t)sum, 0);
            }
            for (uint32_t i : small) {
                uint32_t ax, bx, ay, by, az, bz;
                cell_range(i, 0, ax, bx), cell_range(i, 1, ay, by), cell_range(i, 2, az, bz);
                for (uint32_t z = az; z <= bz; ++z)
                    for (uint32_t y = ay; y <= by; ++y)
                        for (uint32_t x = ax; x <= bx; ++x) {
                            if (!reaches(i, x, y, z)) continue;
                            const uint32_t c = (z * g.ny + y) * g.nx + x;
                            if (pass == 0) {
                                ++count[c];
                            } else {
                                uint32_t& rec = out.cells[c];
                                out.refs[(rec >> RT_GRID_CNT_BITS) + (rec & RT_GRID_CNT_MASK)] = (unsigned short)i;
                                ++rec;
                            }
                        }
            }
        }
        if (out.cells.empty()) continue;
        out.refs_per_sphere = (double)out.refs.size() / (double)small.size();
        if (g.n_cells < 64u || (double)out.refs.size() > 4.0 * (double)g.n_cells || out.refs_per_sphere > 32.0) break;
        g.all_rec = ((uint32_t)out.refs.size() << RT_GRID_CNT_BITS) | n;
        for (uint32_t i = 0; i < n; ++i) out.refs.push_back((unsigned short)i);
        if (out.refs.size() & 1u) out.refs.push_back(0);
        g.n_refs = (uint32_t)out.refs.size();
        g.n_always = (uint32_t)always.size();
        for (uint32_t k = 0; k < g.n_always; ++k) g.always[k] = always[k];
        g.max_coord = (float)(pad * 1048576.0);
        g.n_spheres = n;
        if (grid_lds_bytes(n, g.n_cells, g.n_refs) > lds_budget) continue;
        out.gp = g;
        out.ok = true;
        return;
    }
    out = HostGrid{};
}

__device__ __forceinline__ float min_raw(float a, float b) {
    float r;
    asm("v_min_f32 %0, %1, %2" : "=v"(r) : "v"(a), "v"(b));
    return r;
}
template <bool ONE_LAYER, bool MOTION>
__device__ __forceinline__ void intersect_grid_body(const GridParams& G, const float4* __restrict__ qa,
                                                    const float4* __restrict__ qb, float2* __restrict__ qh,
                                                    const uint32_t* __restrict__ in_counts, const IntersectParams& ip,
                                                    const GenParams* __restrict__ gpd) {
    extern __shared__ __attribute__((aligned(16))) char smem[];
    constexpr uint32_t BLOCK = RT_BVH_BLOCK;
    uint32_t pre[RT_ISECT_MAX_SHARDS + 1];
    pre[0] = 0;
    uint32_t n_my = 0;
#pragma unroll
    for (uint32_t k = 0; k < RT_ISECT_MAX_SHARDS; ++k) {
        const uint32_t q = ip.q0 + blockIdx.x + k * gridDim.x;
        const uint32_t c = q < ip.q1 ? in_counts[q] : 0u;
        pre[k + 1] = pre[k] + c;
        if (q < ip.q1) n_my = k + 1;
    }
    const uint32_t total = pre[RT_ISECT_MAX_SHARDS];
    if (total == 0) return;
    float4* s_geo = reinterpret_cast<float4*>(smem);
    uint32_t* s_cells = reinterpret_cast<uint32_t*>(s_geo + G.n_spheres);
    unsigned short* s_refs = reinterpret_cast<unsigned short*>(s_cells + G.n_cells);
    uint32_t* s_work = reinterpret_cast<uint32_t*>(smem + grid_lds_bytes(G.n_spheres, G.n_cells, G.n_refs) - 16u);
    for (uint32_t i = threadIdx.x; i < G.n_spheres; i += BLOCK) s_geo[i] = G.sph_geo[i];
    float4* s_dc = reinterpret_cast<float4*>(smem + grid_lds_bytes(G.n_spheres, G.n_cells, G.n_refs));
    if (MOTION)
        for (uint32_t i = threadIdx.x; i < G.n_spheres; i += BLOCK) s_dc[i] = gen_motion_of(gpd).sph_dc[i];
    float tm = 0.0f;
    for (uint32_t i = threadIdx.x; i < G.n_cells; i += BLOCK) s_cells[i] = G.cells[i];
    {
        const uint32_t* src = reinterpret_cast<const uint32_t*>(G.refs);
        uint32_t* dst = reinterpret_cast<uint32_t*>(s_refs);
        for (uint32_t i = threadIdx.x; i < G.n_refs / 2u; i += BLOCK) dst[i] = src[i];
    }
    if (threadIdx.x == 0) *s_work = 0u;
    __syncthreads();
    const uint32_t lane = threadIdx.x & 63u;
    const int stride_y = (int)G.nx, stride_z = (int)(G.nx * G.ny);
    const uint32_t last_cell = G.n_cells - 1u;
    const uint32_t all_cnt = G.all_rec & RT_GRID_CNT_MASK, all_off = G.all_rec >> RT_GRID_CNT_BITS;
    bool exhausted = false;
    bool has = false;
    V3 o = splat(0.0f), d = v3(0.f, 0.f, 1.f);
    SharedRcp rcp_a{1.0f, 1.0f};
    float tbest = RT_FLT_MAX, texit = 0.0f;
    float tmx = 0.f, tmy = 0.f, tmz = 0.f, tdx = 0.f, tdy = 0.f, tdz = 0.f;
    int hit = -1, cell = 0, sx = 1, sy = 1, sz = 1;
    uint32_t cnt = 0u, off = 0u, budget = 0u;
    size_t pos = 0;
    auto test_sphere = [&](uint32_t s) {
        float th;
        if (sphere_root(MOTION ? sphere_at(s_geo[s], s_dc[s], tm) : s_geo[s], o, d, rcp_a, 1e-3f, RT_FLT_MAX, th) && (th < tbest || (th == tbest && (int)s > hit))) {
            tbest = th;
            hit = (int)s;
        }
    };
    uint32_t cur_k = 0u, cur_lo = 0u, cur_hi = pre[1];
    size_t cur_base = (size_t)(ip.q0 + blockIdx.x) * ip.cap;
    auto q_finish = [&]() {
        qh[pos] = make_float2(tbest, __int_as_float(hit));
        has = false;
    };
    for (;;) {
        const unsigned long long idle = __ballot(!has);
        const uint32_t n_idle = (uint32_t)__popcll(idle);
        RT_LANE_STAT(0, has);
        if (n_idle >= RT_GRID_REFILL_MIN && !exhausted) {
            RT_LANE_STAT(6, !has);
            uint32_t v0 = 0;
            if (lane == 0) v0 = atomicAdd(s_work, n_idle);
            v0 = __builtin_amdgcn_readfirstlane(v0);
            if (v0 + n_idle >= total) exhausted = true;
            const uint32_t v =
                v0 + __builtin_amdgcn_mbcnt_hi((uint32_t)(idle >> 32), __builtin_amdgcn_mbcnt_lo((uint32_t)idle, 0u));
            while (v0 >= cur_hi && cur_k + 1u < n_my) {
                ++cur_k;
                cur_lo = cur_hi;
                uint32_t nh = total;
#pragma unroll
                for (uint32_t t = 1; t < RT_ISECT_MAX_SHARDS; ++t) nh = (cur_k + 1u == t) ? pre[t] : nh;
                cur_hi = nh;
                cur_base = (size_t)(ip.q0 + blockIdx.x + cur_k * gridDim.x) * ip.cap - cur_lo;
            }
            if (!has && v < total) {
                if (min(v0 + n_idle, total) <= cur_hi) {
                    pos = cur_base + v;
#ifdef RT_DEBUG_QUEUE_BOUNDS
                    if (v - cur_lo >= ip.cap || ip.q0 + blockIdx.x + cur_k * gridDim.x >= ip.q1) __builtin_trap();
#endif
                } else {
                    uint32_t k = 0;
#pragma unroll
                    for (uint32_t t = 1; t < RT_ISECT_MAX_SHARDS; ++t) k += (t < n_my && v >= pre[t]) ? 1u : 0u;
                    uint32_t qoff = v;
#pragma unroll
                    for (uint32_t t = 1; t < RT_ISECT_MAX_SHARDS; ++t) qoff = (k == t) ? v - pre[t] : qoff;
                    const uint32_t shard = ip.q0 + blockIdx.x + k * gridDim.x;
                    pos = (size_t)shard * ip.cap + qoff;
#ifdef RT_DEBUG_QUEUE_BOUNDS
                    if (qoff >= ip.cap || shard >= ip.q1) __builtin_trap();
#endif
                }
                const float4 ra = qa[RT_QSTRIDE * pos], rb = RT_QSTRIDE == 2u ? qa[RT_QSTRIDE * pos + 1u] : qb[RT_QSTRIDE * pos];
                o = v3(ra.x, ra.y, ra.z);
                d = v3(rb.x, rb.y, rb.z);
                rcp_a = shared_rcp(length_squared(d));
                if (MOTION) {
                    uint32_t k0, k1;
                    path_key_of_slot(*gpd, __float_as_uint(ra.w), k0, k1);
                    tm = path_time(gen_motion_of(gpd), k0, k1);
                }
                tbest = RT_FLT_MAX;
                hit = -1;
                has = true;
#pragma unroll
                for (uint32_t k2 = 0; k2 < RT_GRID_MAX_ALWAYS; ++k2)
                    if (k2 < G.n_always) test_sphere(G.always[k2]);
                const float ix = __builtin_amdgcn_rcpf(d.x), iy = __builtin_amdgcn_rcpf(d.y), iz = __builtin_amdgcn_rcpf(d.z);
                const float x0 = (G.g0[0] - o.x) * ix, x1 = (G.b1[0] - o.x) * ix;
                const float y0 = (G.g0[1] - o.y) * iy, y1 = (G.b1[1] - o.y) * iy;
                const float z0 = (G.g0[2] - o.z) * iz, z1 = (G.b1[2] - o.z) * iz;
                const float tn = fmaxf(fmaxf(fminf(x0, x1), fminf(y0, y1)), fmaxf(fminf(z0, z1), 0.0f));
                const float tf = fminf(fminf(fmaxf(x0, x1), fmaxf(y0, y1)), fmaxf(z0, z1));
                const float mo = fmaxf(fmaxf(fabsf(o.x), fabsf(o.y)), fabsf(o.z));
                cnt = 0u;
                if (__builtin_expect(!(mo <= G.max_coord), 0)) {
                    for (uint32_t k = 0; k < all_cnt; ++k) test_sphere(s_refs[all_off + k]);
                    q_finish();
                } else if (!(tn <= tf) || !(tn < tbest)) {
                    qh[pos] = make_float2(tbest, __int_as_float(hit));
                    has = false;
                } else {
                    const float px = __builtin_fmaf(d.x, tn, o.x), py = __builtin_fmaf(d.y, tn, o.y), pz = __builtin_fmaf(d.z, tn, o.z);
                    const float fx = min_raw(fmaxf(floorf((px - G.g0[0]) * G.inv_cs[0]), 0.0f), (float)(G.nx - 1u));
                    const float fy = ONE_LAYER ? 0.0f : min_raw(fmaxf(floorf((py - G.g0[1]) * G.inv_cs[1]), 0.0f), (float)(G.ny - 1u));
                    const float fz = min_raw(fmaxf(floorf((pz - G.g0[2]) * G.inv_cs[2]), 0.0f), (float)(G.nz - 1u));
                    cell = ONE_LAYER ? (int)fz * (int)G.nx + (int)fx : ((int)fz * (int)G.ny + (int)fy) * (int)G.nx + (int)fx;
                    const bool wx = fabsf(ix) < 1e30f, wy = fabsf(iy) < 1e30f, wz = fabsf(iz) < 1e30f;
                    const float bx = __builtin_fmaf(fx + (d.x >= 0.0f ? 1.0f : 0.0f), G.cs[0], G.g0[0]);
                    const float by = __builtin_fmaf(fy + (d.y >= 0.0f ? 1.0f : 0.0f), G.cs[1], G.g0[1]);
                    const float bz = __builtin_fmaf(fz + (d.z >= 0.0f ? 1.0f : 0.0f), G.cs[2], G.g0[2]);
                    tmx = wx ? (bx - o.x) * ix : INFINITY, tdx = wx ? G.cs[0] * fabsf(ix) : INFINITY;
                    if (!ONE_LAYER) tmy = wy ? (by - o.y) * iy : INFINITY, tdy = wy ? G.cs[1] * fabsf(iy) : INFINITY;
                    tmz = wz ? (bz - o.z) * iz : INFINITY, tdz = wz ? G.cs[2] * fabsf(iz) : INFINITY;
                    sx = d.x >= 0.0f ? 1 : -1, sy = d.y >= 0.0f ? stride_y : -stride_y, sz = d.z >= 0.0f ? stride_z : -stride_z;
                    texit = tf;
                    budget = G.nx + G.ny + G.nz;
                    const uint32_t rec = s_cells[cell];
                    cnt = rec & RT_GRID_CNT_MASK, off = rec >> RT_GRID_CNT_BITS;
                }
            }
        }
        if (!__any(has)) {
            if (exhausted) break;
            continue;
        }
        RT_LANE_STAT(2, has && cnt == 0u);
        if (has && cnt == 0u) {
            const float tnext = ONE_LAYER ? min_raw(tmx, tmz) : min_raw(min_raw(tmx, tmy), tmz);
            if (!(tnext < min_raw(tbest, texit))) {
                qh[pos] = make_float2(tbest, __int_as_float(hit));
                has = false;
            } else {
                const bool ax = tmx <= tnext, ay = !ONE_LAYER && !ax && tmy <= tnext, az = !ax && !ay;
                cell += ax ? sx : (ay ? sy : sz);
                tmx = ax ? tmx + tdx : tmx;
                if (!ONE_LAYER) tmy = ay ? tmy + tdy : tmy;
                tmz = az ? tmz + tdz : tmz;
                const uint32_t rec = s_cells[min((uint32_t)cell, last_cell)];
                cnt = rec & RT_GRID_CNT_MASK, off = rec >> RT_GRID_CNT_BITS;
                if (__builtin_expect(--budget == 0u, 0)) {
                    for (uint32_t k = 0; k < all_cnt; ++k) test_sphere(s_refs[all_off + k]);
                    q_finish();
                    cnt = 0u;
                }
            }
        }
        RT_LANE_STAT(4, has && cnt > 0u);
        if (has && cnt > 0u) {
            const uint32_t s = s_refs[off];
            ++off, --cnt;
            test_sphere(s);
        }
    }
}
template <bool ONE_LAYER>
__global__ __launch_bounds__(RT_BVH_BLOCK, 8) void k_intersect_grid(GridParams G, const float4* __restrict__ qa,
                                                                      const float4* __restrict__ qb, float2* __restrict__ qh,
                                                                      const uint32_t* __restrict__ in_counts, IntersectParams ip) {
    intersect_grid_body<ONE_LAYER, false>(G, qa, qb, qh, in_counts, ip, nullptr);
}
template <bool ONE_LAYER>
__global__ __launch_bounds__(RT_BVH_BLOCK, 8) void k_intersect_grid_motion(GridParams G, const float4* __restrict__ qa,
                                                                             const float4* __restrict__ qb, float2* __restrict__ qh,
                                                                             const uint32_t* __restrict__ in_counts, IntersectParams ip,
                                                                             const GenParams* __restrict__ gpd) {
    intersect_grid_body<ONE_LAYER, true>(G, qa, qb, qh, in_counts, ip, gpd);
}

}
```

### ray_tracing_in_one_weekend_amd/csrc/rt_kernels.h

```cpp
#pragma once
#include "rt_device.h"

namespace rt {

#ifndef RT_QSTRIDE
#define RT_QSTRIDE 2u
#endif
struct Queue {
    float4* a;
    float4* b;
    float2* c;
};
#ifndef RT_RAD_FLOATS
#define RT_RAD_FLOATS 3
#endif
__device__ __forceinline__ void rad_store(float* __restrict__ rad, size_t slot, float x, float y, float z) {
    if (RT_RAD_FLOATS == 4) *reinterpret_cast<float4*>(rad + 4u * slot) = make_float4(x, y, z, 0.0f);
    else *reinterpret_cast<float3*>(rad + 3u * slot) = make_float3(x, y, z);
}

struct GenParams {
    float cam_origin[3], cam_horizontal[3], cam_vertical[3], cam_llc[3];
    uint32_t nx, ny;
    uint32_t npix;
    uint32_t n_rays;
    uint32_t s0;
    uint32_t shard_band, shard_count, shard_id;
    uint32_t nq, cap;
    uint32_t seed_lo, seed_hi;
    const uint4* lists;
    const uint32_t* n_overflow;
    float inv_npix, inv_nx, inv_band;
    uint32_t tiles_per_row, tile_pixels;
    float inv_tpr;
};
struct GenLens {
    float lu[3], lv[3];
    float focus_dist;
    float grow;
    float sin_tilt;
};
__device__ __forceinline__ const GenLens& gen_lens_of(const GenParams* gpd) { return *reinterpret_cast<const GenLens*>(gpd + 1); }
struct GenMotion {
    const float4* sph_dc;
    float open, span;
};
#define RT_MOTION_OFFSET 40u
static_assert(sizeof(GenLens) <= RT_MOTION_OFFSET && sizeof(GenParams) % 8u == 0u, "GenMotion behind GenLens");
__device__ __forceinline__ const GenMotion& gen_motion_of(const GenParams* gpd) {
    return *reinterpret_cast<const GenMotion*>(reinterpret_cast<const char*>(gpd + 1) + RT_MOTION_OFFSET);
}
struct GenPlanar {
    const float4* pq;
    uint32_t base, n;
};
#define RT_PLANAR_OFFSET (RT_MOTION_OFFSET + 16u)
static_assert(sizeof(GenMotion) <= 16u && sizeof(GenPlanar) == 16u, "GenPlanar behind GenMotion");
__device__ __forceinline__ const GenPlanar& gen_planar_of(const GenParams* gpd) {
    return *reinterpret_cast<const GenPlanar*>(reinterpret_cast<const char*>(gpd + 1) + RT_PLANAR_OFFSET);
}
#define RT_TIME_COUNTER 254u
__device__ __forceinline__ float path_time(const GenMotion& gm, uint32_t k0, uint32_t k1) {
    Rng rng(k0, k1, RT_TIME_COUNTER);
    return gm.open + rng.next() * gm.span;
}

__device__ __forceinline__ uint32_t udiv_inv(uint32_t x, uint32_t d, float inv, uint32_t& rem) {
    uint32_t qt = (uint32_t)((float)x * inv);
    uint32_t r = x - qt * d;
    if (r >= d) ++qt, r -= d;
    if (r >= d) ++qt, r -= d;
    rem = r;
    return qt;
}
__device__ __forceinline__ void pixel_of_local(const GenParams& gp, uint32_t pl, uint32_t& i, uint32_t& lj) {
    if (gp.tiles_per_row == 0u) {
        lj = udiv_inv(pl, gp.nx, gp.inv_nx, i);
        return;
    }
    if (pl >= gp.tile_pixels) {
        lj = udiv_inv(pl, gp.nx, gp.inv_nx, i);
        return;
    }
    uint32_t tx;
    const uint32_t ty = udiv_inv(pl >> 6, gp.tiles_per_row, gp.inv_tpr, tx);
    i = tx * 8u + (pl & 7u);
    lj = ty * 8u + ((pl >> 3) & 7u);
}
__host__ __device__ inline uint32_t local_of_pixel(uint32_t nx, uint32_t tiles_per_row, uint32_t tile_pixels, uint32_t i, uint32_t lj) {
    if (tiles_per_row == 0u || lj * nx >= tile_pixels) return lj * nx + i;
// ... 909 lines not shown
}

__device__ __forceinline__ void closest_hit_planar(const GenPlanar& gq, V3 o, V3 d, float& tbest, int& hit) {
    for (uint32_t i = 0; i < gq.n; ++i) {
        float th;
        if (planar_root(gq.pq + 5u * i, o, d, 1e-3f, tbest, th)) {
            tbest = th;
            hit = (int)(gq.base + i);
        }
    }
}

__global__ __launch_bounds__(256) void k_intersect_list_planar(DevScene sc, const float4* __restrict__ qa, const float4* __restrict__ qb,
                                                               float2* __restrict__ qh, const uint32_t* __restrict__ in_counts,
                                                               IntersectParams ip, const GenParams* __restrict__ gpd) {
    const uint32_t q = ip.q0 + blockIdx.x;
    const uint32_t count = in_counts[q];
    const size_t qbase = (size_t)q * ip.cap;
    const GenPlanar gq = gen_planar_of(gpd);
    for (uint32_t i = threadIdx.x; i < count; i += 256u) {
        const float4 ra = qa[RT_QSTRIDE * (qbase + i)], rb = qb[RT_QSTRIDE * (qbase + i)];
        const V3 o = v3(ra.x, ra.y, ra.z), d = v3(rb.x, rb.y, rb.z);
        float tbest = RT_FLT_MAX;
        int hit = -1;
        closest_hit_spheres_general(sc, o, d, tbest, hit);
        MediumCtx mc{0u, 0u, depth_counter_base(ip.depth)};
        if (sc.n_media) path_key_of_slot(*gpd, __float_as_uint(ra.w), mc.k0, mc.k1);
        closest_hit_rects(sc, o, d, mc, tbest, hit);
        closest_hit_planar(gq, o, d, tbest, hit);
        qh[qbase + i] = make_float2(tbest, __int_as_float(hit));
    }
}

struct ShadeParams {
    uint32_t nq, cap;
    int depth, max_depth;
    uint32_t sort;
    uint32_t russian_roulette;
    uint32_t q0;
};

#ifdef RT_PROFILE_PHASES
__device__ unsigned long long g_phase_stats[16];
#define RT_PHASE_CLOCK() __builtin_amdgcn_s_memtime()
#else
#define RT_PHASE_CLOCK() 0ull
#endif

#define RT_PERLIN_LDS_MAX_SETS 4u
#ifndef RT_SORT_N
#define RT_SORT_N 512u
#endif
#define RT_NCLASS 64u
#define RT_CLASS_LDS_MAX 4096u
#define RT_SHADE_WAVE_LDS (RT_NCLASS * 4u + RT_SORT_N * 8u + RT_SORT_N * 2u)
__host__ __device__ inline size_t shade_lds_bytes(uint32_t n_entries, uint32_t n_perlin_lds, uint32_t n_fused_spheres, bool sort) {
    size_t b = 16u;
    if (sort) b += 4u * RT_SHADE_WAVE_LDS;
    if (sort && n_entries <= RT_CLASS_LDS_MAX) b += ((size_t)n_entries + 15u) & ~(size_t)15u;
    b += (size_t)n_perlin_lds * (4096u + 1536u);
    b += (size_t)n_fused_spheres * 16u;
    return (b + 15u) & ~(size_t)15u;
}
template <bool PERLIN_LDS, bool GEN, bool RECTS, bool NEST = false, bool LENS = false, bool MOTION = false, bool PLANAR = false>
#ifndef RT_GEN_WAVES
#define RT_GEN_WAVES 4
#endif
#ifndef RT_SORTED_WAVES
#define RT_SORTED_WAVES 4
#endif
__global__ __launch_bounds__(256, GEN ? RT_GEN_WAVES : RT_SORTED_WAVES) void k_shade(DevScene sc, Queue qin, const float2* __restrict__ qh, Queue qout,
                                               const uint32_t* __restrict__ in_counts, uint32_t* __restrict__ out_counts,
                                               float* __restrict__ rad, ShadeParams tp,
                                               unsigned long long* __restrict__ stats,
                                               const GenParams* __restrict__ gpd) {
    extern __shared__ __attribute__((aligned(16))) char smem[];
    const uint32_t q = tp.q0 + blockIdx.x;
    const uint32_t count = in_counts[q];
    if (count == 0) return;
    uint32_t* s_out = reinterpret_cast<uint32_t*>(smem);
    const uint32_t lane = threadIdx.x & 63u;
    const uint32_t w = __builtin_amdgcn_readfirstlane(threadIdx.x >> 6);
    const bool sort = !GEN && tp.sort != 0u;
    size_t lds_off = 16u;
    uint32_t* s_hist = reinterpret_cast<uint32_t*>(smem + lds_off + (size_t)w * RT_SHADE_WAVE_LDS);
    float2* s_rec = reinterpret_cast<float2*>(s_hist + RT_NCLASS);
    unsigned short* s_pos = reinterpret_cast<unsigned short*>(s_rec + RT_SORT_N);
    const uint8_t* cls = sc.sph_class;
    if (sort) {
        lds_off += 4u * RT_SHADE_WAVE_LDS;
        const uint32_t n_ent = sc.n_prims + sc.n_media + (PLANAR ? gen_planar_of(gpd).n : 0u);
        if (n_ent <= RT_CLASS_LDS_MAX) {
            uint8_t* lc = reinterpret_cast<uint8_t*>(smem + lds_off);
            for (uint32_t i = threadIdx.x; i < n_ent; i += 256u) lc[i] = sc.sph_class[i];
            cls = lc;
            lds_off += ((size_t)n_ent + 15u) & ~(size_t)15u;
        }
    }
    PerlinTables pt{sc.perlin_vec, sc.perlin_perm2};
    if (PERLIN_LDS) {
        float4* lv = reinterpret_cast<float4*>(smem + lds_off);
        unsigned short* lp = reinterpret_cast<unsigned short*>(lv + sc.n_perlin * 256u);
        for (uint32_t i = threadIdx.x; i < sc.n_perlin * 256u; i += 256u) lv[i] = sc.perlin_vec[i];
        for (uint32_t i = threadIdx.x; i < sc.n_perlin * 768u; i += 256u) lp[i] = sc.perlin_perm2[i];
        pt = PerlinTables{lv, lp};
        lds_off += (size_t)sc.n_perlin * (4096u + 1536u);
    }
    const bool fused = GEN && !RECTS && gpd->lists != nullptr;
    const float4* s_geo = reinterpret_cast<const float4*>(smem + lds_off);
    if (fused) {
        float4* g = reinterpret_cast<float4*>(smem + lds_off);
        for (uint32_t i = threadIdx.x; i < sc.n_spheres; i += 256u) g[i] = sc.sph_geo[i];
        if (MOTION)
            for (uint32_t i = threadIdx.x; i < sc.n_spheres; i += 256u) g[sc.n_spheres + i] = gen_motion_of(gpd).sph_dc[i];
    }
    const float4* s_dc = s_geo + sc.n_spheres;
    if (threadIdx.x == 0) *s_out = 0u;
    __syncthreads();
    uint32_t n_fetch = 0, n_bad = 0;
    const size_t qbase = (size_t)q * tp.cap;
#ifdef RT_PROFILE_PHASES
    unsigned long long ph[10] = {};
    const unsigned long long ph_t0 = RT_PHASE_CLOCK();
#endif
    const uint32_t bs = count >= 4u * RT_SORT_N ? RT_SORT_N : ((count + 255u) / 256u) * 64u;
    for (uint32_t base = w * bs; base < count; base += 4u * bs) {
        const uint32_t n_here = min(bs, count - base);
#ifdef RT_PROFILE_PHASES
        const unsigned long long ph_a0 = RT_PHASE_CLOCK();
        asm volatile("s_waitcnt vmcnt(0)" ::: "memory");
        const unsigned long long ph_a = RT_PHASE_CLOCK();
        ph[8] += ph_a - ph_a0;
#endif
        if (sort) {
            s_hist[lane] = 0u;
            __builtin_amdgcn_fence(__ATOMIC_ACQ_REL, "workgroup");
            float2 h[RT_SORT_N / 64u];
            uint32_t kr[RT_SORT_N / 64u];
            __builtin_amdgcn_s_waitcnt(0x0F70);
#pragma unroll
            for (uint32_t k = 0; k < RT_SORT_N / 64u; ++k) {
                const uint32_t j = k * 64u + lane;
                h[k] = j < n_here ? qh[qbase + base + j] : make_float2(0.0f, 0.0f);
            }
#ifdef RT_PROFILE_PHASES
            asm volatile("s_waitcnt vmcnt(0)" ::: "memory");
            ph[9] += RT_PHASE_CLOCK() - ph_a;
#endif
#pragma unroll
            for (uint32_t k = 0; k < RT_SORT_N / 64u; ++k) {
                const uint32_t j = k * 64u + lane;
                kr[k] = 0u;
                if (j < n_here) {
                    const int hit = __float_as_int(h[k].y);
#ifdef RT_DEBUG_QUEUE_BOUNDS
                    if (hit >= (int)(sc.n_prims + sc.n_media + (PLANAR ? gen_planar_of(gpd).n : 0u))) __builtin_trap();
#endif
                    const uint32_t key = hit < 0 ? sc.key_miss : (uint32_t)cls[hit];
                    kr[k] = key | (atomicAdd(&s_hist[key], 1u) << 8);
                }
            }
            __builtin_amdgcn_fence(__ATOMIC_ACQ_REL, "workgroup");
            {
                const uint32_t v = s_hist[lane];
                uint32_t incl = v;
#pragma unroll
                for (int off = 1; off < 64; off <<= 1) {
                    const uint32_t t = __shfl_up(incl, off);
                    if ((int)lane >= off) incl += t;
                }
                __builtin_amdgcn_fence(__ATOMIC_ACQ_REL, "workgroup");
                s_hist[lane] = incl - v;
            }
            __builtin_amdgcn_fence(__ATOMIC_ACQ_REL, "workgroup");
#pragma unroll
            for (uint32_t k = 0; k < RT_SORT_N / 64u; ++k) {
                const uint32_t j = k * 64u + lane;
                if (j < n_here) {
                    const uint32_t dst = s_hist[kr[k] & 255u] + (kr[k] >> 8);
                    s_rec[dst] = h[k];
                    s_pos[dst] = (unsigned short)j;
                }
            }
            __builtin_amdgcn_fence(__ATOMIC_ACQ_REL, "workgroup");
        }
        float2 hA = make_float2(0.0f, 0.0f), rcA = hA;
        float4 raA = make_float4(0.f, 0.f, 0.f, 0.f), rbA = raA;
        auto fetch = [&](uint32_t seg, float2& h, float4& ra, float4& rb, float2& rc) {
            const uint32_t j = seg + lane;
            if (!GEN && j < n_here) {
                uint32_t pj = j;
                if (sort) h = s_rec[j], pj = s_pos[j];
                else h = qh[qbase + base + j];
                const size_t r = qbase + base + pj;
                ra = qin.a[RT_QSTRIDE * r], rb = qin.b[RT_QSTRIDE * r], rc = qin.c[r];
            }
        };
        fetch(0u, hA, raA, rbA, rcA);
#ifdef RT_PROFILE_PHASES
        const unsigned long long ph_b = RT_PHASE_CLOCK();
        asm volatile("s_waitcnt vmcnt(0)" ::: "memory");
        unsigned long long ph_c = RT_PHASE_CLOCK();
        ph[1] += ph_b - ph_a, ph[2] += ph_c - ph_b, ph[5] += 1;
#endif
        for (uint32_t seg = 0; seg < n_here; seg += 64u) {
            float2 hB = make_float2(0.0f, 0.0f), rcB = hB;
            float4 raB = make_float4(0.f, 0.f, 0.f, 0.f), rbB = raB;
            bool prefetched = false;
            auto prefetch = [&]() {
                if (!prefetched && seg + 64u < n_here) fetch(seg + 64u, hB, raB, rbB, rcB);
                prefetched = true;
            };
            const uint32_t j = seg + lane;
            RT_LANE_STAT(18, j < n_here);
            if (!GEN && __all(j >= n_here || __float_as_int(hA.y) < 0)) {
                if (j < n_here) {
                    const V3 d = v3(rbA.x, rbA.y, rbA.z);
                    V3 Lr = splat(0.0f);
                    if (!near_one(d)) ++n_bad;
                    else Lr = v3(rbA.w, rcA.x, rcA.y) * sky_value(sc, d, n_fetch);
                    rad_store(rad, __float_as_uint(raA.w), Lr.x, Lr.y, Lr.z);
                }
                prefetch();
                hA = hB, raA = raB, rbA = rbB, rcA = rcB;
#ifdef RT_PROFILE_PHASES
                { const unsigned long long t = RT_PHASE_CLOCK(); ph[3] += t - ph_c, ph[6] += 1, ph_c = t; }
#endif
                continue;
            }
            bool alive = false;
            Bounce bo;
            bo.o = bo.d = bo.attenuation = splat(0.0f);
            V3 T = splat(0.0f);
            float rr_threshold = 0.0f;
            uint32_t slot = 0, k0 = 0, k1 = 0;
            float tm = 0.0f;
            if (j < n_here) {
                float2 h = hA;
                V3 o, d;
                if (GEN) {
                    uint32_t pl;
                    slot = primary_idx_of(tp.nq, q, base + j);
                    gen_primary<LENS>(*gpd, gen_lens_of(gpd), slot, o, d, k0, k1, pl);
                    if (MOTION) tm = path_time(gen_motion_of(gpd), k0, k1);
                    T = splat(1.0f);
                    uint4 list = make_uint4(RT_LIST_OVERFLOW, 0u, 0u, 0u);
                    if (fused) list = gpd->lists[pl];
                    const uint32_t n_list = list.x & 0xFFFFu;
                    RT_LANE_STAT(14, fused && n_list != RT_LIST_OVERFLOW);
                    if (fused && n_list != RT_LIST_OVERFLOW) {
                        const SharedRcp ra = shared_rcp(length_squared(d));
                        float tbest = RT_FLT_MAX;
                        int hit = -1;
                        const uint32_t ids[RT_LIST_MAX] = {list.x >> 16, list.y & 0xFFFFu, list.y >> 16, list.z & 0xFFFFu,
                                                           list.z >> 16, list.w & 0xFFFFu, list.w >> 16};
#pragma unroll
                        for (uint32_t t = 0; t < RT_LIST_MAX; ++t) {
                            float th;
                            const int s = (int)ids[t];
                            if (t < n_list) RT_LANE_STAT(12, true);
                            if (t < n_list && sphere_root(MOTION ? sphere_at(s_geo[s], s_dc[s], tm) : s_geo[s], o, d, ra, 1e-3f, RT_FLT_MAX, th) &&
                                (th < tbest || (th == tbest && s > hit))) {
                                tbest = th;
                                hit = s;
                            }
                        }
                        h = make_float2(tbest, __int_as_float(hit));
                    } else {
                        h = qh[qbase + base + j];
                    }
                } else {
                    o = v3(raA.x, raA.y, raA.z), d = v3(rbA.x, rbA.y, rbA.z);
                    T = v3(rbA.w, rcA.x, rcA.y);
                    slot = __float_as_uint(raA.w);
                    path_key_of_slot(*gpd, slot, k0, k1);
                    if (MOTION) tm = path_time(gen_motion_of(gpd), k0, k1);
                }
                V3 Lr = splat(0.0f);
                if (!near_one(d)) {
                    ++n_bad;
                } else {
#ifdef RT_DEBUG_QUEUE_BOUNDS
                    if (__float_as_int(h.y) >= (int)(sc.n_prims + sc.n_media + (PLANAR ? gen_planar_of(gpd).n : 0u))) __builtin_trap();
#endif
                    Rng rng{k0, k1, depth_counter_base(tp.depth)};
                    bo = shade<RECTS, decltype(prefetch), NEST, MOTION, PLANAR>(sc, pt, o, d, __float_as_int(h.y), h.x, rng, n_fetch, prefetch,
                                                                                MOTION ? gen_motion_of(gpd).sph_dc : nullptr, tm,
                                                                                PLANAR ? gen_planar_of(gpd).pq : nullptr,
                                                                                PLANAR ? gen_planar_of(gpd).base : 0u);
                    if (bo.alive && tp.russian_roulette) {
                        const float rr = rng.next();
                        rr_threshold = fmaxf(bo.attenuation.x, fmaxf(bo.attenuation.y, bo.attenuation.z));
                        if (!(rr < rr_threshold)) bo.alive = false;
                    }
                    if (bo.alive) {
                        alive = tp.depth < tp.max_depth;
                    } else {
                        Lr = T * bo.radiance;
                    }
                }
                if (!alive) rad_store(rad, slot, Lr.x, Lr.y, Lr.z);
            }
            prefetch();
            const unsigned long long mask = __ballot(alive);
            if (mask) {
                uint32_t wbase = 0;
                if (lane == 0) wbase = atomicAdd(s_out, (uint32_t)__popcll(mask));
                wbase = __builtin_amdgcn_readfirstlane(wbase);
                if (alive) {
                    const uint32_t rk =
                        __builtin_amdgcn_mbcnt_hi((uint32_t)(mask >> 32), __builtin_amdgcn_mbcnt_lo((uint32_t)mask, 0u));
                    const size_t pos = qbase + wbase + rk;
#ifdef RT_DEBUG_QUEUE_BOUNDS
                    if (wbase + rk >= tp.cap) __builtin_trap();
#endif
                    V3 Tn = T * bo.attenuation;
                    if (tp.russian_roulette) Tn = Tn / rr_threshold;
                    qout.a[RT_QSTRIDE * pos] = make_float4(bo.o.x, bo.o.y, bo.o.z, __uint_as_float(slot));
                    qout.b[RT_QSTRIDE * pos] = make_float4(bo.d.x, bo.d.y, bo.d.z, Tn.x);
                    qout.c[pos] = make_float2(Tn.y, Tn.z);
// ... 287 lines not shown
```

Before: 30810.

## Retire sky-miss rays inside grid intersect kernel instead of shade kernel

When the grid intersect path is used and the sky is not an environment map, rays that miss have their sky radiance computed and stored directly in the intersect kernel, and are marked with a retired hit code. The shade kernel then drops retired rays from its sort and compaction, so it never fetches their queue records. The aim is to remove the shade-side load and the wavefront work spent on miss rays. In exchange the intersect kernel gains extra registers, a per-ray throughput load and atomics, which could lower its occupancy.

```diff
diff --git a/include/rtow_mi355x_debug.h b/include/rtow_mi355x_debug.h
--- a/include/rtow_mi355x_debug.h
+++ b/include/rtow_mi355x_debug.h
@@ -9,6 +9,7 @@
 
 #define RT_FLAG_TIME_DEPTHS 4u
 #define RT_FLAG_PRODUCTION_KERNELS 8u
+#define RT_FLAG_TINTED_THROUGHPUT 16u
 
 int rt_get_depth_timings(RtCtx* ctx, uint32_t max_n, float* isect_ms, float* shade_ms, uint64_t* rays);
 
@@ -29,7 +30,8 @@
     RT_OPT_MATERIALISE_PRIMARIES = 11,
     RT_OPT_MEDIUM_SEARCH = 12,
     RT_OPT_POOL_CHUNK_DELAY_US = 13,
-    RT_OPT__COUNT = 14
+    RT_OPT_RETIRE_MISSES = 14,
+    RT_OPT__COUNT = 15
 };
 int rt_debug_set_option(RtCtx* ctx, uint32_t option, uint32_t value);
 int rt_debug_get_option(const RtCtx* ctx, uint32_t option, uint32_t* value);
@@ -50,6 +52,8 @@
     uint32_t nest;
 } RtSceneInfo;
 int rt_debug_scene_info(const RtCtx* ctx, RtSceneInfo* info);
+
+int rt_debug_retired_rays(RtCtx* ctx, uint64_t* n_retired, uint64_t* n_bad_dir);
 
 int rt_debug_planar_info(const RtCtx* ctx, uint32_t* n_planar, uint32_t* plane_data_in_lds);
 int rt_debug_planar_bounds(const RtQuads* quads, float world_mag, float* box, float* slack);
diff --git a/ray_tracing_in_one_weekend_amd/_ffi.py b/ray_tracing_in_one_weekend_amd/_ffi.py
--- a/ray_tracing_in_one_weekend_amd/_ffi.py
+++ b/ray_tracing_in_one_weekend_amd/_ffi.py
@@ -10,6 +10,7 @@
 FLAG_BRUTE_FORCE = 1
 FLAG_RUSSIAN_ROULETTE = 2
 FLAG_TIME_DEPTHS = 4
+FLAG_TINTED_THROUGHPUT = 16
 FLAG_PRODUCTION_KERNELS = 8
 RTH_INVALID = 0xFFFFFFFF
 
@@ -105,12 +106,14 @@
 
 MULTI_COPY_GATHER = 1
 (OPT_TREE_PLACEMENT, OPT_PRIMARY_LISTS, OPT_PIXEL_ORDER, OPT_TEXEL_POOL, OPT_GRID, OPT_GRID_CELL, OPT_CHAINS,
- OPT_GENERAL_KERNELS, OPT_GENERAL_LDS, OPT_QUEUE_SHARDS, OPT_ISECT_WORKGROUPS, OPT_MATERIALISE_PRIMARIES, OPT_MEDIUM_SEARCH, OPT_POOL_CHUNK_DELAY_US) = range(14)
+ OPT_GENERAL_KERNELS, OPT_GENERAL_LDS, OPT_QUEUE_SHARDS, OPT_ISECT_WORKGROUPS, OPT_MATERIALISE_PRIMARIES, OPT_MEDIUM_SEARCH, OPT_POOL_CHUNK_DELAY_US,
+ OPT_RETIRE_MISSES) = range(15)
 OPT_NAMES = {"tree_placement": OPT_TREE_PLACEMENT, "primary_lists": OPT_PRIMARY_LISTS, "pixel_order": OPT_PIXEL_ORDER,
              "texel_pool": OPT_TEXEL_POOL, "grid": OPT_GRID, "grid_cell": OPT_GRID_CELL, "chains": OPT_CHAINS,
              "general_kernels": OPT_GENERAL_KERNELS, "general_lds": OPT_GENERAL_LDS, "queue_shards": OPT_QUEUE_SHARDS,
              "isect_workgroups": OPT_ISECT_WORKGROUPS, "materialise_primaries": OPT_MATERIALISE_PRIMARIES,
-             "medium_search": OPT_MEDIUM_SEARCH, "pool_chunk_delay_us": OPT_POOL_CHUNK_DELAY_US}
+             "medium_search": OPT_MEDIUM_SEARCH, "pool_chunk_delay_us": OPT_POOL_CHUNK_DELAY_US,
+             "retire_misses": OPT_RETIRE_MISSES}
 
 
 class RtSceneInfo(C.Structure):
@@ -129,7 +132,7 @@
 GPU_SYMBOLS = ["rt_abi_version", "rt_build_id", "rt_ctx_create", "rt_ctx_destroy", "rt_last_error", "rt_scene_upload",
                "rt_shard_rows", "rt_shard_row_to_image_row", "rt_prepare", "rt_render", "rt_render_device", "rt_debug_bounce", "rt_debug_arithmetic",
                "rt_get_depth_timings", "rt_set_progress", "rt_host_alloc", "rt_host_free", "rt_debug_set_option", "rt_debug_get_option",
-               "rt_debug_scene_info", "rt_debug_grid_build", "rt_debug_world_bounds", "rt_debug_render_parts", "rt_multi_create", "rt_multi_create_ex", "rt_multi_destroy", "rt_multi_device_count",
+               "rt_debug_scene_info", "rt_debug_retired_rays", "rt_debug_grid_build", "rt_debug_world_bounds", "rt_debug_render_parts", "rt_multi_create", "rt_multi_create_ex", "rt_multi_destroy", "rt_multi_device_count",
                "rt_multi_last_error", "rt_multi_scene_upload", "rt_multi_render", "rt_deinterleave_bands", "rt_set_lens", "rt_multi_set_lens",
                "rt_set_motion", "rt_multi_set_motion", "rt_debug_motion_bounds",
                "rt_set_quads", "rt_multi_set_quads", "rt_debug_planar_info", "rt_debug_planar_bounds"]
@@ -219,6 +222,8 @@
     lib.rt_debug_get_option.restype = C.c_int
     lib.rt_debug_scene_info.argtypes = [vp, C.POINTER(RtSceneInfo)]
     lib.rt_debug_scene_info.restype = C.c_int
+    lib.rt_debug_retired_rays.argtypes = [vp, _u64, _u64]
+    lib.rt_debug_retired_rays.restype = C.c_int
     lib.rt_debug_render_parts.argtypes = [vp, C.c_char_p, C.c_uint32]
     lib.rt_debug_render_parts.restype = C.c_int
     lib.rt_debug_grid_build.argtypes = [C.POINTER(RtFlatScene), C.c_uint32, C.c_uint32, C.c_float * 8, C.c_uint32 * 3, _u32, _u32, _u16, _u32,
diff --git a/ray_tracing_in_one_weekend_amd/api.py b/ray_tracing_in_one_weekend_amd/api.py
--- a/ray_tracing_in_one_weekend_amd/api.py
+++ b/ray_tracing_in_one_weekend_amd/api.py
@@ -372,6 +372,13 @@
         d["n_planar"], d["plane_data_in_lds"] = n.value, lds.value
         return d
 
+    def retired_rays(self):
+        n, bad = C.c_uint64(0), C.c_uint64(0)
+        rc = self._lib.rt_debug_retired_rays(self._ctx, C.byref(n), C.byref(bad))
+        if rc != 0:
+            self._raise("rt_debug_retired_rays", rc)
+        return n.value, bad.value
+
     def shard_rows(self, params):
         return self._lib.rt_shard_rows(params.ny, params.shard_band or 1, params.shard_count, params.shard_id)
 
diff --git a/ray_tracing_in_one_weekend_amd/csrc/rt_api.hip b/ray_tracing_in_one_weekend_amd/csrc/rt_api.hip
--- a/ray_tracing_in_one_weekend_amd/csrc/rt_api.hip
+++ b/ray_tracing_in_one_weekend_amd/csrc/rt_api.hip
@@ -66,6 +66,9 @@
     GridParams grid{};
     size_t grid_lds = 0;
     uint32_t opt[RT_OPT__COUNT] = {};
+    const unsigned long long* retired_dev = nullptr;
+    const unsigned long long* bad_dir_dev = nullptr;
+    hipStream_t retired_stream = nullptr;
     uint32_t* h_overflow = nullptr;
     long long last_overflow = -1;
     RtLens lens{0.0f, 1.0f};
@@ -281,6 +284,7 @@
     bool lens = false;
     bool motion = false;
     bool planar = false;
+    unsigned long long* retired = nullptr;
 };
 bool scene_is_general(const RtCtx* ctx) { return ctx->general_kernels; }
 bool grid_enabled(const RtCtx* ctx) { return ctx->use_grid && ctx->opt[RT_OPT_GRID] != 1u && !scene_is_general(ctx); }
@@ -290,10 +294,14 @@
     const bool rects = scene_is_general(ctx);
     if (use_bvh && !gen && grid_enabled(ctx)) {
         const size_t mlds = ctx->grid_lds + ctx->motion_lds;
+        const bool retire = !b.motion && ctx->ds.sky_type != RT_SKY_ENV && ctx->opt[RT_OPT_RETIRE_MISSES] != 1u;
+        const RetireArgs ra{b.rad, b.qi.c, b.totals, b.retired, ctx->ds.sky_type};
         if (b.motion && ctx->grid.ny == 1u) hipLaunchKernelGGL(k_intersect_grid_motion<true>, dim3(grid), dim3(RT_BVH_BLOCK), mlds, sg, ctx->grid, b.qi.a, b.qi.b, b.qhit, b.cin, ip, b.gpd);
         else if (b.motion) hipLaunchKernelGGL(k_intersect_grid_motion<false>, dim3(grid), dim3(RT_BVH_BLOCK), mlds, sg, ctx->grid, b.qi.a, b.qi.b, b.qhit, b.cin, ip, b.gpd);
-        else if (ctx->grid.ny == 1u) hipLaunchKernelGGL(k_intersect_grid<true>, dim3(grid), dim3(RT_BVH_BLOCK), ctx->grid_lds, sg, ctx->grid, b.qi.a, b.qi.b, b.qhit, b.cin, ip);
-        else hipLaunchKernelGGL(k_intersect_grid<false>, dim3(grid), dim3(RT_BVH_BLOCK), ctx->grid_lds, sg, ctx->grid, b.qi.a, b.qi.b, b.qhit, b.cin, ip);
+        else if (retire && ctx->grid.ny == 1u) hipLaunchKernelGGL((k_intersect_grid<true, true>), dim3(grid), dim3(RT_BVH_BLOCK), ctx->grid_lds, sg, ctx->grid, b.qi.a, b.qi.b, b.qhit, b.cin, ip, ra);
+        else if (retire) hipLaunchKernelGGL((k_intersect_grid<false, true>), dim3(grid), dim3(RT_BVH_BLOCK), ctx->grid_lds, sg, ctx->grid, b.qi.a, b.qi.b, b.qhit, b.cin, ip, ra);
+        else if (ctx->grid.ny == 1u) hipLaunchKernelGGL(k_intersect_grid<true>, dim3(grid), dim3(RT_BVH_BLOCK), ctx->grid_lds, sg, ctx->grid, b.qi.a, b.qi.b, b.qhit, b.cin, ip, RetireArgs{});
+        else hipLaunchKernelGGL(k_intersect_grid<false>, dim3(grid), dim3(RT_BVH_BLOCK), ctx->grid_lds, sg, ctx->grid, b.qi.a, b.qi.b, b.qhit, b.cin, ip, RetireArgs{});
         return;
     }
     if (b.planar && use_bvh) {
@@ -791,6 +799,7 @@
             RT_ISECT_VARIANTS(false, true, true),  RT_ISECT_VARIANTS(true, true, true),  RT_ISECT_VARIANTS(false, false, true),  RT_ISECT_VARIANTS(true, false, true),
 #undef RT_ISECT_VARIANTS
             reinterpret_cast<const void*>(&k_intersect_grid<true>), reinterpret_cast<const void*>(&k_intersect_grid<false>),
+            reinterpret_cast<const void*>(&k_intersect_grid<true, true>), reinterpret_cast<const void*>(&k_intersect_grid<false, true>),
             reinterpret_cast<const void*>(&k_debug_bounce<RT_BVH_BLOCK, true, true>),
             reinterpret_cast<const void*>(&k_debug_bounce<RT_BVH_BLOCK, true, false>),
 #define RT_SHADE_VARIANTS(P, G) reinterpret_cast<const void*>(&k_shade<P, G, false>), reinterpret_cast<const void*>(&k_shade<P, G, true>), reinterpret_cast<const void*>(&k_shade<P, G, true, true>)
@@ -1334,7 +1343,7 @@
     if ((rc = ensure(ctx, ctx->acc, (size_t)npix * 3 * sizeof(float)))) return rc;
     const size_t counts_bytes = (size_t)(n_depths + 1) * nq * sizeof(uint32_t);
     if ((rc = ensure(ctx, ctx->counts, counts_bytes))) return rc;
-    const size_t totals_bytes = (size_t)(n_depths + 2) * sizeof(unsigned long long);
+    const size_t totals_bytes = (size_t)(n_depths + 3) * sizeof(unsigned long long);
     if ((rc = ensure(ctx, ctx->totals, totals_bytes))) return rc;
     if ((rc = ensure(ctx, ctx->genp, sizeof(GenParams) + RT_PLANAR_OFFSET + sizeof(GenPlanar)))) return rc;
     if (want_lists &&(rc = ensure(ctx, ctx->lists, ((size_t)npix + 1u) * sizeof(uint4)))) return rc;
@@ -1342,6 +1351,7 @@
     float* acc = (float*)ctx->acc.p;
     uint32_t* counts = (uint32_t*)ctx->counts.p;
     unsigned long long* totals = (unsigned long long*)ctx->totals.p;
+    ctx->retired_dev = totals + n_depths + 2, ctx->bad_dir_dev = totals + 1, ctx->retired_stream = st;
     SlicePlan plan;
     if ((rc = plan_slices(ctx, prm, npix64, plan))) return rc;
     if (const char* e = pool_request(ctx->pool, plan.want_bytes)) return fail(ctx, RT_ERR_NOMEM, std::string("render: ") + e);
@@ -1482,7 +1492,7 @@
             const bool gen = fuse_gen && depth == 0;
             ip.depth = depth;
             ip.q0 = q0, ip.q1 = q1;
-            const StepBuffers sb{qi, qo, qhit, cin, cout, rad, totals, gpd, lens, ctx->motion, ctx->planar};
+            const StepBuffers sb{qi, qo, qhit, cin, cout, rad, totals, gpd, lens, ctx->motion, ctx->planar, totals + n_depths + 2};
             const bool no_primary_trace = gen && !rects && gp.lists != nullptr && no_overflow;
             if (!no_primary_trace) launch_intersect(ctx, sg, use_bvh, gen, isect_grid_g, sb, ip);
             if (td) RT_HIP(ctx, hipEventRecord(ctx->depth_events[3 * (size_t)depth + 1], st));
@@ -1531,7 +1541,7 @@
     if (stats) {
         RT_HIP(ctx, hipStreamSynchronize(st));
         ctx->mark("wait_for_the_device");
-        std::vector<unsigned long long> h((size_t)n_depths + 2);
+        std::vector<unsigned long long> h((size_t)n_depths + 3);
         RT_HIP(ctx, hipMemcpy(h.data(), totals, totals_bytes, hipMemcpyDeviceToHost));
         std::memset(stats, 0, sizeof(*stats));
         stats->n_paths = (uint64_t)npix * spp;
@@ -2169,6 +2179,23 @@
         restore_static_search(ctx);
         ctx->err = err;
         return rc;
+    }
+    return RT_OK;
+}
+
+int rt_debug_retired_rays(RtCtx* ctx, uint64_t* n_retired, uint64_t* n_bad_dir) {
+    if (!ctx || !n_retired) return RT_ERR_INVALID;
+    *n_retired = 0;
+    if (n_bad_dir) *n_bad_dir = 0;
+    if (!ctx->retired_dev) return RT_OK;
+    RT_HIP(ctx, hipSetDevice(ctx->device));
+    RT_HIP(ctx, hipStreamSynchronize(ctx->retired_stream));
+    unsigned long long v = 0;
+    RT_HIP(ctx, hipMemcpy(&v, ctx->retired_dev, sizeof(v), hipMemcpyDeviceToHost));
+    *n_retired = v;
+    if (n_bad_dir) {
+        RT_HIP(ctx, hipMemcpy(&v, ctx->bad_dir_dev, sizeof(v), hipMemcpyDeviceToHost));
+        *n_bad_dir = v;
     }
     return RT_OK;
 }
@@ -2222,9 +2249,17 @@
     if (ctx->motion) hipLaunchKernelGGL(k_set_motion, dim3(1), dim3(64), 0, st, (GenParams*)ctx->genp.p, ctx->gmotion);
     if (ctx->planar) hipLaunchKernelGGL(k_set_planar, dim3(1), dim3(64), 0, st, (GenParams*)ctx->genp.p, ctx->gplanar);
     hipLaunchKernelGGL(k_debug_fill, dim3((n + 255u) / 256u), dim3(256), 0, st, gp, Q[0], d_o, d_d);
+    std::vector<float2> tint;
+    if (io->flags & RT_FLAG_TINTED_THROUGHPUT) {
+        tint.assign((size_t)nq * cap, make_float2(0.5f, 0.25f));
+        RT_HIP(ctx, hipMemcpyAsync(Q[0].c, tint.data(), tint.size() * sizeof(float2), hipMemcpyHostToDevice, st));
+        RT_HIP(ctx, hipStreamSynchronize(st));
+    }
     const bool use_bvh = ctx->use_bvh && !(io->flags & RT_FLAG_BRUTE_FORCE);
     const StepBuffers sb{Q[0], Q[1], wv.qhit, counts, counts + nq, wv.rad,
-                         (unsigned long long*)ctx->totals.p, (const GenParams*)ctx->genp.p, false, ctx->motion, ctx->planar};
+                         (unsigned long long*)ctx->totals.p, (const GenParams*)ctx->genp.p, false, ctx->motion, ctx->planar,
+                         (unsigned long long*)ctx->totals.p + 3};
+    ctx->retired_dev = sb.retired, ctx->bad_dir_dev = sb.totals + 1, ctx->retired_stream = st;
     const IntersectParams ip{nq, cap, (int)io->depth, 0u, nq};
     launch_intersect(ctx, st, use_bvh, false, qg.isect_grid, sb, ip);
     const ShadeParams sp{nq, cap, (int)io->depth, 0x7FFFFFFF, 1u, 0u, 0u};
@@ -2256,7 +2291,8 @@
     for (uint32_t i = 0; i < n; ++i) {
         const uint32_t chunk = i >> 8;
         const size_t pos = (size_t)(chunk % nq) * cap + (size_t)(chunk / nq) * 256u + (i & 255u);
-        const int hit = (int)bits(hh[pos].y);
+        int hit = (int)bits(hh[pos].y);
+        if (hit == RT_HIT_RETIRED) hit = -1;
         io->out_hit[i] = hit;
         io->out_t[i] = hit >= 0 ? hh[pos].x : 0.0f;
         io->out_alive[i] = 0;
diff --git a/ray_tracing_in_one_weekend_amd/csrc/rt_grid.h b/ray_tracing_in_one_weekend_amd/csrc/rt_grid.h
--- a/ray_tracing_in_one_weekend_amd/csrc/rt_grid.h
+++ b/ray_tracing_in_one_weekend_amd/csrc/rt_grid.h
@@ -190,11 +190,18 @@
     asm("v_min_f32 %0, %1, %2" : "=v"(r) : "v"(a), "v"(b));
     return r;
 }
-template <bool ONE_LAYER, bool MOTION>
+struct RetireArgs {
+    float* rad;
+    const float2* qc;
+    unsigned long long* stats;
+    unsigned long long* n_retired;
+    uint32_t sky_type;
+};
+template <bool ONE_LAYER, bool MOTION, bool RETIRE>
 __device__ __forceinline__ void intersect_grid_body(const GridParams& G, const float4* __restrict__ qa,
                                                     const float4* __restrict__ qb, float2* __restrict__ qh,
                                                     const uint32_t* __restrict__ in_counts, const IntersectParams& ip,
-                                                    const GenParams* __restrict__ gpd) {
+                                                    const GenParams* __restrict__ gpd, const RetireArgs& rt) {
     extern __shared__ __attribute__((aligned(16))) char smem[];
     constexpr uint32_t BLOCK = RT_BVH_BLOCK;
     uint32_t pre[RT_ISECT_MAX_SHARDS + 1];
@@ -224,7 +231,7 @@
         uint32_t* dst = reinterpret_cast<uint32_t*>(s_refs);
         for (uint32_t i = threadIdx.x; i < G.n_refs / 2u; i += BLOCK) dst[i] = src[i];
     }
-    if (threadIdx.x == 0) *s_work = 0u;
+    if (threadIdx.x == 0) s_work[0] = 0u, s_work[1] = 0u;
     __syncthreads();
     const uint32_t lane = threadIdx.x & 63u;
     const int stride_y = (int)G.nx, stride_z = (int)(G.nx * G.ny);
@@ -248,9 +255,32 @@
     };
     uint32_t cur_k = 0u, cur_lo = 0u, cur_hi = pre[1];
     size_t cur_base = (size_t)(ip.q0 + blockIdx.x) * ip.cap;
+    bool pending = false;
+    uint32_t slot = 0u;
+    float Tx = 0.0f;
+    uint32_t n_retired = 0u, n_bad = 0u;
+    DevScene sky{};
+    sky.sky_type = rt.sky_type == 0u ? 0u : 1u;
     auto q_finish = [&]() {
-        qh[pos] = make_float2(tbest, __int_as_float(hit));
+        qh[pos] = make_float2(tbest, __int_as_float(RETIRE && hit < 0 ? RT_HIT_RETIRED : hit));
+        if (RETIRE) pending = hit < 0;
         has = false;
+    };
+    auto retire = [&]() {
+        if (!RETIRE) return;
+        const unsigned long long m = __ballot(pending);
+        if (m == 0ull) return;
+        const bool ok = near_one(d);
+        n_retired += (uint32_t)__popcll(m);
+        n_bad += (uint32_t)__popcll(__ballot(pending && !ok));
+        if (pending) {
+            const float2 tc = rt.qc[pos];
+            uint32_t n_fetch = 0u;
+            V3 Lr = splat(0.0f);
+            if (ok) Lr = v3(Tx, tc.x, tc.y) * sky_value(sky, d, n_fetch);
+            rad_store(rt.rad, slot, Lr.x, Lr.y, Lr.z);
+            pending = false;
+        }
     };
     for (;;) {
         const unsigned long long idle = __ballot(!has);
@@ -258,6 +288,7 @@
         RT_LANE_STAT(0, has);
         if (n_idle >= RT_GRID_REFILL_MIN && !exhausted) {
             RT_LANE_STAT(6, !has);
+            retire();
             uint32_t v0 = 0;
             if (lane == 0) v0 = atomicAdd(s_work, n_idle);
             v0 = __builtin_amdgcn_readfirstlane(v0);
@@ -295,6 +326,7 @@
                 const float4 ra = qa[RT_QSTRIDE * pos], rb = RT_QSTRIDE == 2u ? qa[RT_QSTRIDE * pos + 1u] : qb[RT_QSTRIDE * pos];
                 o = v3(ra.x, ra.y, ra.z);
                 d = v3(rb.x, rb.y, rb.z);
+                if (RETIRE) slot = __float_as_uint(ra.w), Tx = rb.w;
                 rcp_a = shared_rcp(length_squared(d));
                 if (MOTION) {
                     uint32_t k0, k1;
@@ -319,8 +351,7 @@
                     for (uint32_t k = 0; k < all_cnt; ++k) test_sphere(s_refs[all_off + k]);
                     q_finish();
                 } else if (!(tn <= tf) || !(tn < tbest)) {
-                    qh[pos] = make_float2(tbest, __int_as_float(hit));
-                    has = false;
+                    q_finish();
                 } else {
                     const float px = __builtin_fmaf(d.x, tn, o.x), py = __builtin_fmaf(d.y, tn, o.y), pz = __builtin_fmaf(d.z, tn, o.z);
                     const float fx = min_raw(fmaxf(floorf((px - G.g0[0]) * G.inv_cs[0]), 0.0f), (float)(G.nx - 1u));
@@ -343,15 +374,17 @@
             }
         }
         if (!__any(has)) {
-            if (exhausted) break;
+            if (exhausted) {
+                retire();
+                break;
+            }
             continue;
         }
         RT_LANE_STAT(2, has && cnt == 0u);
         if (has && cnt == 0u) {
             const float tnext = ONE_LAYER ? min_raw(tmx, tmz) : min_raw(min_raw(tmx, tmy), tmz);
             if (!(tnext < min_raw(tbest, texit))) {
-                qh[pos] = make_float2(tbest, __int_as_float(hit));
-                has = false;
+                q_finish();
             } else {
                 const bool ax = tmx <= tnext, ay = !ONE_LAYER && !ax && tmy <= tnext, az = !ax && !ay;
                 cell += ax ? sx : (ay ? sy : sz);
@@ -374,19 +407,28 @@
             test_sphere(s);
         }
     }
-}
-template <bool ONE_LAYER>
+    if (RETIRE) {
+        if (lane == 0) {
+            if (n_bad) atomicAdd(&rt.stats[1], (unsigned long long)n_bad);
+            if (n_retired) atomicAdd(&s_work[1], n_retired);
+        }
+        __syncthreads();
+        if (threadIdx.x == 0 && s_work[1]) atomicAdd(rt.n_retired, (unsigned long long)s_work[1]);
+    }
+}
+template <bool ONE_LAYER, bool RETIRE = false>
 __global__ __launch_bounds__(RT_BVH_BLOCK, 8) void k_intersect_grid(GridParams G, const float4* __restrict__ qa,
                                                                       const float4* __restrict__ qb, float2* __restrict__ qh,
-                                                                      const uint32_t* __restrict__ in_counts, IntersectParams ip) {
-    intersect_grid_body<ONE_LAYER, false>(G, qa, qb, qh, in_counts, ip, nullptr);
+                                                                      const uint32_t* __restrict__ in_counts, IntersectParams ip,
+                                                                      RetireArgs rt) {
+    intersect_grid_body<ONE_LAYER, false, RETIRE>(G, qa, qb, qh, in_counts, ip, nullptr, rt);
 }
 template <bool ONE_LAYER>
 __global__ __launch_bounds__(RT_BVH_BLOCK, 8) void k_intersect_grid_motion(GridParams G, const float4* __restrict__ qa,
                                                                              const float4* __restrict__ qb, float2* __restrict__ qh,
                                                                              const uint32_t* __restrict__ in_counts, IntersectParams ip,
                                                                              const GenParams* __restrict__ gpd) {
-    intersect_grid_body<ONE_LAYER, true>(G, qa, qb, qh, in_counts, ip, gpd);
-}
-
-}
+    intersect_grid_body<ONE_LAYER, true, false>(G, qa, qb, qh, in_counts, ip, gpd, RetireArgs{});
+}
+
+}
diff --git a/ray_tracing_in_one_weekend_amd/csrc/rt_kernels.h b/ray_tracing_in_one_weekend_amd/csrc/rt_kernels.h
--- a/ray_tracing_in_one_weekend_amd/csrc/rt_kernels.h
+++ b/ray_tracing_in_one_weekend_amd/csrc/rt_kernels.h
@@ -6,6 +6,7 @@
 #ifndef RT_QSTRIDE
 #define RT_QSTRIDE 2u
 #endif
+#define RT_HIT_RETIRED (-2)
 struct Queue {
     float4* a;
     float4* b;
@@ -1081,6 +1082,7 @@
     const uint32_t lane = threadIdx.x & 63u;
     const uint32_t w = __builtin_amdgcn_readfirstlane(threadIdx.x >> 6);
     const bool sort = !GEN && tp.sort != 0u;
+    constexpr bool RETIRED = !GEN && !RECTS && !MOTION && !PLANAR;
     size_t lds_off = 16u;
     uint32_t* s_hist = reinterpret_cast<uint32_t*>(smem + lds_off + (size_t)w * RT_SHADE_WAVE_LDS);
     float2* s_rec = reinterpret_cast<float2*>(s_hist + RT_NCLASS);
@@ -1125,6 +1127,7 @@
     const uint32_t bs = count >= 4u * RT_SORT_N ? RT_SORT_N : ((count + 255u) / 256u) * 64u;
     for (uint32_t base = w * bs; base < count; base += 4u * bs) {
         const uint32_t n_here = min(bs, count - base);
+        uint32_t n_live = n_here;
 #ifdef RT_PROFILE_PHASES
         const unsigned long long ph_a0 = RT_PHASE_CLOCK();
         asm volatile("s_waitcnt vmcnt(0)" ::: "memory");
@@ -1155,8 +1158,12 @@
 #ifdef RT_DEBUG_QUEUE_BOUNDS
                     if (hit >= (int)(sc.n_prims + sc.n_media + (PLANAR ? gen_planar_of(gpd).n : 0u))) __builtin_trap();
 #endif
-                    const uint32_t key = hit < 0 ? sc.key_miss : (uint32_t)cls[hit];
-                    kr[k] = key | (atomicAdd(&s_hist[key], 1u) << 8);
+                    if (RETIRED && hit == RT_HIT_RETIRED) {
+                        kr[k] = 255u;
+                    } else {
+                        const uint32_t key = hit < 0 ? sc.key_miss : (uint32_t)cls[hit];
+                        kr[k] = key | (atomicAdd(&s_hist[key], 1u) << 8);
+                    }
                 }
             }
             __builtin_amdgcn_fence(__ATOMIC_ACQ_REL, "workgroup");
@@ -1170,12 +1177,13 @@
                 }
                 __builtin_amdgcn_fence(__ATOMIC_ACQ_REL, "workgroup");
                 s_hist[lane] = incl - v;
+                if (RETIRED) n_live = (uint32_t)__builtin_amdgcn_readlane((int)incl, 63);
             }
             __builtin_amdgcn_fence(__ATOMIC_ACQ_REL, "workgroup");
 #pragma unroll
             for (uint32_t k = 0; k < RT_SORT_N / 64u; ++k) {
                 const uint32_t j = k * 64u + lane;
-                if (j < n_here) {
+                if (j < n_here && (!RETIRED || (kr[k] & 255u) != 255u)) {
                     const uint32_t dst = s_hist[kr[k] & 255u] + (kr[k] >> 8);
                     s_rec[dst] = h[k];
                     s_pos[dst] = (unsigned short)j;
@@ -1187,7 +1195,7 @@
         float4 raA = make_float4(0.f, 0.f, 0.f, 0.f), rbA = raA;
         auto fetch = [&](uint32_t seg, float2& h, float4& ra, float4& rb, float2& rc) {
             const uint32_t j = seg + lane;
-            if (!GEN && j < n_here) {
+            if (!GEN && j < n_live) {
                 uint32_t pj = j;
                 if (sort) h = s_rec[j], pj = s_pos[j];
                 else h = qh[qbase + base + j];
@@ -1202,18 +1210,19 @@
         unsigned long long ph_c = RT_PHASE_CLOCK();
         ph[1] += ph_b - ph_a, ph[2] += ph_c - ph_b, ph[5] += 1;
 #endif
-        for (uint32_t seg = 0; seg < n_here; seg += 64u) {
+        for (uint32_t seg = 0; seg < n_live; seg += 64u) {
             float2 hB = make_float2(0.0f, 0.0f), rcB = hB;
             float4 raB = make_float4(0.f, 0.f, 0.f, 0.f), rbB = raB;
             bool prefetched = false;
             auto prefetch = [&]() {
-                if (!prefetched && seg + 64u < n_here) fetch(seg + 64u, hB, raB, rbB, rcB);
+                if (!prefetched && seg + 64u < n_live) fetch(seg + 64u, hB, raB, rbB, rcB);
                 prefetched = true;
             };
             const uint32_t j = seg + lane;
-            RT_LANE_STAT(18, j < n_here);
-            if (!GEN && __all(j >= n_here || __float_as_int(hA.y) < 0)) {
-                if (j < n_here) {
+            const bool live = j < n_live && (!RETIRED || sort || __float_as_int(hA.y) != RT_HIT_RETIRED);
+            RT_LANE_STAT(18, live);
+            if (!GEN && __all(!live || __float_as_int(hA.y) < 0)) {
+                if (live) {
                     const V3 d = v3(rbA.x, rbA.y, rbA.z);
                     V3 Lr = splat(0.0f);
                     if (!near_one(d)) ++n_bad;
@@ -1234,7 +1243,7 @@
             float rr_threshold = 0.0f;
             uint32_t slot = 0, k0 = 0, k1 = 0;
             float tm = 0.0f;
-            if (j < n_here) {
+            if (live) {
                 float2 h = hA;
                 V3 o, d;
                 if (GEN) {
```

New measurement: 28520. 0.926x the previous value.
